# wzhe06/SparrowRecSys

Hardware: AMD Instinct MI355X
Metric: ctr_samples_per_sec (higher is better)
Workload: dtype f32

## Files before the change

### sparrowrecsys_amd/csrc/api_forward.h

```cpp
static int launch_din_cols(sprk_handle h, const int32_t* ids, float* pooled, float* att, int32_t B, const DinColsMany* many, hipStream_t st) {
    DinColsRun c = h->din_cols_run;
    const long long ntasks = (long long)(many ? many->n : 1) * ((B + 15) / 16);
    const long long slots = (long long)h->num_cus * 16;
    c.ts = (c.T >= 16 && ntasks * 4 <= slots) ? 4 : ((c.T >= 8 && ntasks * 2 <= slots) ? 2 : 1);
    if (h->tune.din_cols_ts) c.ts = h->tune.din_cols_ts;
    if (many) c.ts = 1;
    c.ts_log2 = c.ts == 4 ? 2 : (c.ts == 2 ? 1 : 0);
    c.ql = (c.T + 3) / 4;
    const int EL = 4 * h->din_cols_kc;
    const size_t lds = ((size_t)2 * 64 * 36 + (size_t)DC_WAVES * 16 * c.idp + (size_t)DC_WAVES * 2 * 64 * EL) * sizeof(float);
    const long long grid = (ntasks * c.ts + DC_WAVES - 1) / DC_WAVES;
    if (many) {
        if (h->din_cols_kc == 2)
            hipLaunchKernelGGL((k_din_attn_cols<2, true>), dim3((unsigned)grid), dim3(DC_WAVES * 64), lds, st, c, (const int*)nullptr, (float*)nullptr, (float*)nullptr, B, h->dev_err, *many);
        else
            hipLaunchKernelGGL((k_din_attn_cols<1, true>), dim3((unsigned)grid), dim3(DC_WAVES * 64), lds, st, c, (const int*)nullptr, (float*)nullptr, (float*)nullptr, B, h->dev_err, *many);
    } else {
        if (h->din_cols_kc == 2)
            hipLaunchKernelGGL((k_din_attn_cols<2, false>), dim3((unsigned)grid), dim3(DC_WAVES * 64), lds, st, c, ids, pooled, att, B, h->dev_err, DinColsOne{});
        else
            hipLaunchKernelGGL((k_din_attn_cols<1, false>), dim3((unsigned)grid), dim3(DC_WAVES * 64), lds, st, c, ids, pooled, att, B, h->dev_err, DinColsOne{});
    }
    HIP_TRY(hipGetLastError());
    return SPRK_OK;
}

static int launch_din_fused(sprk_handle h, const int32_t* ids, const float* dense, float* out, float* att, int32_t B, const DinFusedMany* many,
                            bool tail, hipStream_t st) {
    DinFusedRun c = h->din_fused_run;
    const long long ntasks = (long long)(many ? many->n : 1) * ((B + 15) / 16);
    const long long slots = (long long)h->num_cus * DF_WAVES;
    c.ts = (c.T >= 16 && ntasks * 4 <= slots) ? 4 : ((c.T >= 8 && ntasks * 2 <= slots) ? 2 : 1);
    if (h->tune.din_cols_ts) c.ts = h->tune.din_cols_ts;
    c.ts_log2 = c.ts == 4 ? 2 : (c.ts == 2 ? 1 : 0);
    c.ql = ((c.T + 3) / 4 + 3) & ~3;
    const int kc = h->din_cols_kc;
    const size_t lds = ((size_t)DF_COEF_FLOATS + (tail ? (size_t)DinFusedImg::dma_floats : 0) + (size_t)DF_WAVES * 16 * c.idp +
                        (size_t)DF_WAVES * (tail ? 1 : 2) * 64 * 4 * kc) * sizeof(float);
    long long grid = (ntasks * c.ts + DF_WAVES - 1) / DF_WAVES;
    if (many && grid > h->num_cus) grid = h->num_cus;
#define DF_LAUNCH(KC, MB, TAIL, marg)                                                                                                   \
    hipLaunchKernelGGL((k_din_fused<KC, MB, TAIL>), dim3((unsigned)grid), dim3(DF_WAVES * 64), lds, st, c, MB ? (const int*)nullptr : ids, \
                       MB ? (const float*)nullptr : dense, MB ? (float*)nullptr : out, MB ? (float*)nullptr : att, B, h->dev_err, marg)
    if (many) {
        if (kc == 2) { if (tail) DF_LAUNCH(2, true, true, *many); else DF_LAUNCH(2, true, false, *many); }
        else { if (tail) DF_LAUNCH(1, true, true, *many); else DF_LAUNCH(1, true, false, *many); }
    } else {
        if (att && !tail) {
            if (kc == 2) hipLaunchKernelGGL((k_din_fused<2, false, false, true>), dim3((unsigned)grid), dim3(DF_WAVES * 64), lds, st, c, ids, dense, out, att, B, h->dev_err, DinFusedOne{});
            else hipLaunchKernelGGL((k_din_fused<1, false, false, true>), dim3((unsigned)grid), dim3(DF_WAVES * 64), lds, st, c, ids, dense, out, att, B, h->dev_err, DinFusedOne{});
        } else if (kc == 2) { if (tail) DF_LAUNCH(2, false, true, DinFusedOne{}); else DF_LAUNCH(2, false, false, DinFusedOne{}); }
        else { if (tail) DF_LAUNCH(1, false, true, DinFusedOne{}); else DF_LAUNCH(1, false, false, DinFusedOne{}); }
    }
#undef DF_LAUNCH
    HIP_TRY(hipGetLastError());
    return SPRK_OK;
}

static int launch_din(sprk_handle h, const int32_t* ids, float* pooled, float* att, int32_t B, hipStream_t st) {
    if (att && (h->stage == Stage::DienSeq || h->stage == Stage::DienSeqMfma)) return fail(SPRK_EINVAL, "DIEN stage has no attention output");
    switch (h->stage) {
    case Stage::DinFusedAttn: return launch_din_fused(h, ids, nullptr, pooled, att, B, nullptr, false, st);
    case Stage::DinCols: return launch_din_cols(h, ids, pooled, att, B, nullptr, st);
    case Stage::DinPool: {
        const int nchunks = (B + h->din_ms - 1) / h->din_ms;
        const int grid = nchunks < h->din_grid_cap ? nchunks : h->din_grid_cap;
        hipLaunchKernelGGL(k_din_pool, dim3(grid), dim3(256), h->din_lds_bytes, st, h->dev_plan, ids, pooled, att, B, h->din_ms, h->dev_err);
        break;
    }
    case Stage::DienSeqMfma: {
        DienRun run = h->dien_run;
        run.image = h->dien_frag;
        const int ntiles = (B + 15) / 16;
        int gridm = (ntiles + DM_WAVES - 1) / DM_WAVES;
        if (gridm > h->num_cus * 8) gridm = h->num_cus * 8;
        const size_t lds10 = DienFrag<10, 32>::total_pad * sizeof(float), lds16 = DienFrag<16, 32>::total_pad * sizeof(float);
        if (h->plan.din.emb_dim == 10)
            hipLaunchKernelGGL((k_dien_seq_mfma<10, 32>), dim3(gridm), dim3(DM_WAVES * 64), lds10, st, run, ids, pooled, B, h->dev_err);
        else
            hipLaunchKernelGGL((k_dien_seq_mfma<16, 32>), dim3(gridm), dim3(DM_WAVES * 64), lds16, st, run, ids, pooled, B, h->dev_err);
        break;
    }
    case Stage::DienSeq: {
        int grid = (B + 63) / 64;
        if (grid > h->num_cus * 8) grid = h->num_cus * 8;
        if (h->plan.din.emb_dim == 10)
            hipLaunchKernelGGL((k_dien_seq<10, 32>), dim3(grid), dim3(64), 0, st, h->dien_run, ids, pooled, B, h->dev_err);
        else
            hipLaunchKernelGGL((k_dien_seq<16, 32>), dim3(grid), dim3(64), 0, st, h->dien_run, ids, pooled, B, h->dev_err);
        break;
    }
    case Stage::None: return fail(SPRK_EKIND, "handle has no DIN stage");
    }
    HIP_TRY(hipGetLastError());
    return SPRK_OK;
}

static int din_tail_waves(sprk_handle h) {
    return h->din_tail_run.e_unscale != 0.f ? dt_waves_unf(kDinTailVariants[h->din_tail_variant].kpc) : DT_WAVES;
}

int sprk_din_pool(sprk_handle h, const int32_t* ids, float* pooled, float* att, int32_t B, void* stream) {
    RoctxRange roctx_range_("sprk_din_pool");
    if (!h || !ids || !pooled) return fail(SPRK_EINVAL, "NULL argument");
    if (!h->finalized) return fail(SPRK_ESTATE, "din_pool before finalize");
    if (!h->plan.din.enabled) return fail(SPRK_EKIND, "handle has no DIN stage");
    if (B <= 0) return B == 0 ? SPRK_OK : fail(SPRK_EINVAL, "negative batch");
    return launch_din(h, ids, pooled, att, B, (hipStream_t)stream);
}

int sprk_forward(sprk_handle h, const int32_t* ids, const float* dense, float* out, int32_t B,
                 void* workspace, size_t workspace_bytes, void* stream) {
    RoctxRange roctx_range_("sprk_forward");
    if (!h) return fail(SPRK_EINVAL, "handle is NULL");
    if (!h->finalized) return fail(SPRK_ESTATE, "forward before finalize");
    if (B < 0) return fail(SPRK_EINVAL, "negative batch");
    if (B == 0) return SPRK_OK;
    if (!out) return fail(SPRK_EINVAL, "out is NULL");
    if (h->plan.n_id_cols > 0 && !ids) return fail(SPRK_EINVAL, "ids is NULL");
    if (h->plan.n_dense > 0 && !dense) return fail(SPRK_EINVAL, "dense is NULL");
    hipStream_t st = (hipStream_t)stream;
    const float* aux = nullptr;
    if (h->plan.din.enabled) {
        const size_t need = sprk_workspace_bytes(h, B);
        if (!workspace || workspace_bytes < need) return fail(SPRK_EINVAL, "workspace too small: %zu < %zu bytes", workspace_bytes, need);
        if (h->route == Route::DinFused) {
            if ((long long)((B + 15) / 16) <= (long long)h->num_cus * DF_WAVES) return launch_din_fused(h, ids, dense, out, nullptr, B, nullptr, true, st);
            DinFusedMany fm;
            memset(&fm, 0, sizeof(fm));
            fm.n = 1; fm.ids[0] = ids; fm.dense[0] = dense; fm.out[0] = out;
            return launch_din_fused(h, nullptr, nullptr, nullptr, nullptr, B, &fm, true, st);
        }
        if (h->route == Route::DienFused) {
            DienRun run = h->dien_run;
            run.image = h->dien_frag;
            const int ntiles = (B + 15) / 16;
            int grid = (ntiles + DNF_WAVES - 1) / DNF_WAVES;
            if (grid > h->num_cus) grid = h->num_cus;
            if (h->plan.din.emb_dim == 10)
                hipLaunchKernelGGL((k_dien_fused<10, 32, 8, 4>), dim3(grid), dim3(DNF_WAVES * 64), h->dien_fused_lds, st, run, h->din_tail_run, ids, dense, out, B,
                                   h->dev_err, (const float*)h->din_tail_image, (float*)workspace);
            else
                hipLaunchKernelGGL((k_dien_fused<16, 32, 8, 4>), dim3(grid), dim3(DNF_WAVES * 64), h->dien_fused_lds, st, run, h->din_tail_run, ids, dense, out, B,
                                   h->dev_err, (const float*)h->din_tail_image, (float*)workspace);
            HIP_TRY(hipGetLastError());
            return SPRK_OK;
        }
        SPRK_TRY(launch_din(h, ids, (float*)workspace, nullptr, B, st));
        aux = (const float*)workspace;
    }
    const int ntasks = (B + 15) / 16;
    const int unaligned = (((uintptr_t)ids | (uintptr_t)dense) & 15) ? 1 : 0;
    switch (h->route) {
    case Route::V2Joint: {
        const V2JVariant& jv = kV2JVariants[h->v2j_variant];
        V2JRun jr = h->v2j_run;
        jr.flags = unaligned;
        const V2J1Variant* one = nullptr;
        if (h->v2j1_image && ntasks <= V2J1_MAX_TASKS)
            for (const V2J1Variant& v : kV2J1Variants)
                if (!one && v.g_big == jv.g_big && v.njf == jv.njf) one = &v;
        if (one) {
            (h->v2j1_hoist ? one->launch_h : one->launch)(jr, ids, dense, out, B, h->dev_err, h->v2j1_image, (ntasks + h->v2j1_waves - 1) / h->v2j1_waves,
                                                          h->v2j1_lds_bytes, st);
            break;
        }
        int grid = (ntasks + V2_WAVES - 1) / V2_WAVES;
        if (grid > h->v2_grid_cap) grid = h->v2_grid_cap;
        jv.launch(jr, ids, dense, out, B, h->dev_err, h->v2_image, grid, h->v2j_lds_bytes, st);
        break;
    }
    case Route::Rows: {
        int grid = (ntasks + RC_WAVES - 1) / RC_WAVES;
        if (grid > h->num_cus) grid = h->num_cus;
        RowsRun rr = h->rows_run;
        rr.flags = unaligned;
        if (h->rows_one && ntasks <= V2J1_MAX_TASKS)
            kRowsVariants[h->rows_variant].launch_one(rr, ids, dense, out, B, h->dev_err, h->rows_image, (ntasks + RC_WAVES - 1) / RC_WAVES,
                                                      h->rows_lds_bytes, st);
        else
            kRowsVariants[h->rows_variant].launch(rr, ids, dense, out, B, h->dev_err, h->rows_image, grid, h->rows_lds_bytes, st);
        break;
    }
    case Route::Pairs: {
        int grid = (ntasks + V1_WAVES - 1) / V1_WAVES;
        if (grid > h->num_cus) grid = h->num_cus;
        if (h->v1_one && ntasks <= V1_ONE_MAX_TASKS)
            kV1Variants[h->v1_variant].launch_one(h->v1_run, ids, dense, out, B, h->dev_err, (ntasks + V1_WAVES - 1) / V1_WAVES, st);
        else
            kV1Variants[h->v1_variant].launch(h->v1_run, ids, dense, out, B, h->dev_err, grid, st);
        break;
    }
    case Route::MlpRows: {
        int grid = (ntasks + MR_WAVES - 1) / MR_WAVES;
        if (grid > h->num_cus) grid = h->num_cus;
        MlpRowsRun rr = h->mlp_rows_run;
        rr.flags = (rr.flags & ~1) | unaligned;
        hipLaunchKernelGGL(h->mlp_rows_kernel, dim3(grid), dim3(MR_WAVES * 64), h->mlp_rows_lds, st, rr, ids, dense, out, B, h->dev_err, (const float*)h->mlp_rows_image);
        break;
    }
    case Route::DinTail: {
        const int tw = din_tail_waves(h);
        int grid = (ntasks + tw - 1) / tw;
        if (grid > h->num_cus) grid = h->num_cus;
        kDinTailVariants[h->din_tail_variant].launch(h->din_tail_run, ids, dense, aux, out, B, h->dev_err, h->din_tail_image, grid, st);
        break;
    }
    default: {
        const int ntiles = (B + SPRK_TILE_M - 1) / SPRK_TILE_M;
        const int grid = ntiles < h->tile_grid_cap ? ntiles : h->tile_grid_cap;
        hipLaunchKernelGGL(k_tile_forward, dim3(grid), dim3(256), h->tile_lds_bytes, st, h->dev_plan, ids, dense, aux, out, B, h->dev_err);
    }
    }
    HIP_TRY(hipGetLastError());
    return SPRK_OK;
}

static int fork_helpers(sprk_handle h, int S, hipStream_t st) {
    HIP_TRY(hipEventRecord(h->many_fork, st));
    for (int s = 0; s < S; ++s) HIP_TRY(hipStreamWaitEvent(h->many_stream[s], h->many_fork, 0));
    return SPRK_OK;
}
static int join_helpers(sprk_handle h, int S, hipStream_t st) {
    for (int s = 0; s < S; ++s) {
        HIP_TRY(hipEventRecord(h->many_join[s], h->many_stream[s]));
        HIP_TRY(hipStreamWaitEvent(st, h->many_join[s], 0));
    }
    return SPRK_OK;
}

extern "C++" {
template <class Many, class Launch>
static int launch_groups(int32_t n_batches, int per, const int32_t* const* ids, const float* const* dense, float* const* out, Launch launch) {
    int g = 0;
    for (int32_t i0 = 0; i0 < n_batches; i0 += per, ++g) {
        Many m;
        memset(&m, 0, sizeof(m));
        m.n = n_batches - i0 < per ? n_batches - i0 : per;
        for (int j = 0; j < m.n; ++j) { m.ids[j] = ids[i0 + j]; m.dense[j] = dense ? dense[i0 + j] : nullptr; m.out[j] = out[i0 + j]; }
        SPRK_TRY(launch(m, g));
        HIP_TRY(hipGetLastError());
    }
    return SPRK_OK;
}
template <class Ok> static bool every_batch(int32_t n_batches, Ok ok) {
    for (int32_t i = 0; i < n_batches; ++i)
        if (!ok(i)) return false;
    return true;
}
}

static int forward_many_impl(sprk_handle h, int32_t n_batches, const int32_t* const* ids, const float* const* dense,
                             float* const* out, int32_t B, void* workspace, size_t workspace_bytes, void* stream,
                             int many_batches, int many_streams) {
    RoctxRange roctx_range_("sprk_forward_many");
    if (!h) return fail(SPRK_EINVAL, "handle is NULL");
    if (n_batches < 0) return fail(SPRK_EINVAL, "negative batch count");
    if (n_batches > 0 && !out) return fail(SPRK_EINVAL, "out is NULL");
    int S = (h->finalized && n_batches > 1) ? many_streams : 0;
    const size_t ws_need = (sprk_workspace_bytes(h, B) + 255) & ~(size_t)255;
    const bool ws_untouched = h->finalized && (h->route == Route::DinFused || h->route == Route::DienFused);
    if (S >= 2 && ws_need > 0 && !ws_untouched) {
        while (S >= 2 && (!workspace || workspace_bytes < (size_t)S * ws_need)) --S;
        if (S < 2) S = 0;
    }
    hipStream_t st = (hipStream_t)stream;
    const bool grouped = h->finalized && many_batches > 1 && n_batches > 1 && B > 0 && ids;
    const int ntpb = (B + 15) / 16;
    auto aligned = [&](int32_t i, const float* d) { return !(((uintptr_t)ids[i] | (uintptr_t)d) & 15); };
    auto present = [&](int32_t i) { return ids[i] && dense[i] && out[i]; };
    if (grouped && dense && h->route == Route::V2Joint && every_batch(n_batches, [&](int32_t i) { return present(i) && aligned(i, dense[i]); })) {
        const V2JVariant& jv = kV2JVariants[h->v2j_variant];
        V2JRun jr = h->v2j_run;
        jr.flags = 0;
        return launch_groups<V2JMany>(n_batches, many_batches, ids, dense, out, [&](V2JMany& m, int) {
            m.ntpb = ntpb;
            long long grid = ((long long)m.n * ntpb + V2_WAVES - 1) / V2_WAVES;
            if (grid > h->v2_grid_cap) grid = h->v2_grid_cap;
            jv.launch_many(jr, m, B, h->dev_err, h->v2_image, (int)grid, h->v2j_lds_bytes, st);
            return SPRK_OK;
        });
    }
    const float* const* rows_dense = h->plan.n_dense ? dense : nullptr;
    if (grouped && (dense || h->plan.n_dense == 0) && h->route == Route::Rows &&
        every_batch(n_batches, [&](int32_t i) { return ids[i] && out[i] && (!rows_dense || rows_dense[i]) && aligned(i, rows_dense ? rows_dense[i] : nullptr); })) {
        const RowsVariant& rv = kRowsVariants[h->rows_variant];
        RowsRun rr = h->rows_run;
        rr.flags = 0;
        return launch_groups<RowsMany>(n_batches, many_batches < RC_MB ? many_batches : RC_MB, ids, rows_dense, out, [&](RowsMany& m, int) {
            m.ntpb = ntpb;
            long long grid = ((long long)m.n * ntpb + RC_WAVES - 1) / RC_WAVES;
            if (grid > h->num_cus) grid = h->num_cus;
            rv.launch_many(rr, m, B, h->dev_err, h->rows_image, (int)grid, h->rows_lds_bytes, st);
            return SPRK_OK;
        });
    }
    if (grouped && dense && h->route == Route::MlpRows && h->mlp_rows_many_kernel &&
        every_batch(n_batches, [&](int32_t i) { return present(i) && aligned(i, dense[i]); })) {
        MlpRowsRun rr = h->mlp_rows_run;
        rr.flags &= ~1;
        return launch_groups<MlpRowsMany>(n_batches, many_batches < MR_MB ? many_batches : MR_MB, ids, dense, out, [&](MlpRowsMany& m, int) {
            long long grid = ((long long)m.n * ntpb + MR_WAVES - 1) / MR_WAVES;
            if (grid > h->num_cus) grid = h->num_cus;
            hipLaunchKernelGGL(h->mlp_rows_many_kernel, dim3((int)grid), dim3(MR_WAVES * 64), h->mlp_rows_lds, st, rr, m, B, h->dev_err,
                               (const float*)h->mlp_rows_image);
            return SPRK_OK;
        });
    }
    if (grouped && dense && h->route == Route::Pairs && every_batch(n_batches, present)) {
        const V1Variant& vv = kV1Variants[h->v1_variant];
        return launch_groups<V1Many>(n_batches, many_batches < V1_MB ? many_batches : V1_MB, ids, dense, out, [&](V1Many& m, int) {
            m.ntpb = ntpb;
            long long grid = ((long long)m.n * ntpb + V1_WAVES - 1) / V1_WAVES;
            if (grid > h->num_cus) grid = h->num_cus;
            vv.launch_many(h->v1_run, m, B, h->dev_err, (int)grid, st);
            return SPRK_OK;
        });
    }
    if (grouped && dense && h->route == Route::DinFused && h->tune.din_fused_mb && every_batch(n_batches, present)) {
        const int SG = S >= 2 ? S : 1;
        if (SG >= 2) SPRK_TRY(fork_helpers(h, SG, st));
        SPRK_TRY(launch_groups<DinFusedMany>(n_batches, many_batches < DF_MB ? many_batches : DF_MB, ids, dense, out, [&](DinFusedMany& m, int g) {
            return launch_din_fused(h, nullptr, nullptr, nullptr, nullptr, B, &m, true, SG >= 2 ? h->many_stream[g % SG] : st);
        }));
        if (SG >= 2) SPRK_TRY(join_helpers(h, SG, st));
        return SPRK_OK;
    }
    const bool cols = h->stage == Stage::DinCols || h->stage == Stage::DinFusedAttn;
    if (grouped && dense && workspace && ws_need > 0 && cols && (h->route == Route::DinTail || h->route == Route::DinFused)) {
        int per = many_batches < DIN_MB ? many_batches : DIN_MB;
        if ((size_t)per * ws_need > workspace_bytes) per = (int)(workspace_bytes / ws_need);
        if (per >= 2 && every_batch(n_batches, present)) {
            int SG = S >= 2 ? S : 1;
            while (SG > 1 && (size_t)SG * per * ws_need > workspace_bytes) --SG;
            if (SG >= 2) SPRK_TRY(fork_helpers(h, SG, st));
            const DinTailVariant& tv = kDinTailVariants[h->din_tail_variant];
            const int tw = din_tail_waves(h);
            int g = 0;
            for (int32_t i0 = 0; i0 < n_batches; i0 += per, ++g) {
                const int n = n_batches - i0 < per ? n_batches - i0 : per;
                hipStream_t sg = SG >= 2 ? h->many_stream[g % SG] : st;
                char* wbase = (char*)workspace + (size_t)(g % SG) * per * ws_need;
                DinTailMany tm;
                memset(&tm, 0, sizeof(tm));
                tm.n = n; tm.ntpb = ntpb;
                for (int j = 0; j < n; ++j) {
                    float* pooled = (float*)(wbase + (size_t)j * ws_need);
                    tm.ids[j] = ids[i0 + j]; tm.dense[j] = dense[i0 + j]; tm.aux[j] = pooled; tm.out[j] = out[i0 + j];
                }
                if (n <= DC_MB) {
                    DinColsMany cm;
                    memset(&cm, 0, sizeof(cm));
                    cm.n = n;
                    for (int j = 0; j < n; ++j) { cm.ids[j] = tm.ids[j]; cm.pooled[j] = const_cast<float*>(tm.aux[j]); }
                    SPRK_TRY(launch_din_cols(h, nullptr, nullptr, nullptr, B, &cm, sg));
                } else {
                    for (int j = 0; j < n; ++j) SPRK_TRY(launch_din_cols(h, tm.ids[j], const_cast<float*>(tm.aux[j]), nullptr, B, nullptr, sg));
                }
                long long tg = ((long long)n * ntpb + tw - 1) / tw;
                if (tg > h->num_cus) tg = h->num_cus;
                tv.launch_many(h->din_tail_run, tm, B, h->dev_err, h->din_tail_image, (int)tg, sg);
                HIP_TRY(hipGetLastError());
            }
            if (SG >= 2) SPRK_TRY(join_helpers(h, SG, st));
            return SPRK_OK;
        }
    }
    if (S >= 2) SPRK_TRY(fork_helpers(h, S, st));
    for (int32_t i = 0; i < n_batches; ++i) {
        const bool sliced = S >= 2 && ws_need > 0 && !ws_untouched;
        void* wsi = sliced ? (void*)((char*)workspace + (size_t)(i % S) * ws_need) : workspace;
        SPRK_TRY(sprk_forward(h, ids ? ids[i] : nullptr, dense ? dense[i] : nullptr, out[i], B, wsi,
                              sliced ? ws_need : workspace_bytes, S >= 2 ? (void*)h->many_stream[i % S] : stream));
    }
    if (S >= 2) SPRK_TRY(join_helpers(h, S, st));
    return SPRK_OK;
}

int sprk_forward_many(sprk_handle h, int32_t n_batches, const int32_t* const* ids, const float* const* dense,
                      float* const* out, int32_t B, void* workspace, size_t workspace_bytes, void* stream) {
    if (!h) return fail(SPRK_EINVAL, "handle is NULL");
    return forward_many_impl(h, n_batches, ids, dense, out, B, workspace, workspace_bytes, stream, h->many_batches, h->many_streams);
}

int sprk_forward_many_opts(sprk_handle h, int32_t n_batches, const int32_t* const* ids, const float* const* dense,
                           float* const* out, int32_t B, void* workspace, size_t workspace_bytes, void* stream,
                           int32_t batches_per_launch, int32_t helper_streams) {
    if (!h) return fail(SPRK_EINVAL, "handle is NULL");
    if (batches_per_launch < 1 || batches_per_launch > V2J_MB) return fail(SPRK_EINVAL, "batches per launch %d outside [1,%d]", batches_per_launch, V2J_MB);
    if (helper_streams < 0 || helper_streams > 4) return fail(SPRK_EINVAL, "stream count %d outside [0,4]", helper_streams);
    return forward_many_impl(h, n_batches, ids, dense, out, B, workspace, workspace_bytes, stream, batches_per_launch,
                             helper_streams < 2 ? 0 : helper_streams);
}

#define SPRK_FORWARD_KIND(name, kind)                                                                      \
    int name(sprk_handle h, const int32_t* ids, const float* dense, float* out, int32_t B, void* ws,      \
             size_t ws_bytes, void* stream) {                                                              \
        if (!h) return fail(SPRK_EINVAL, "handle is NULL");                                                \
        if (h->plan.model_kind != kind) return fail(SPRK_EKIND, #name ": handle holds model kind %d", h->plan.model_kind); \
        return sprk_forward(h, ids, dense, out, B, ws, ws_bytes, stream);                                  \
    }
SPRK_FORWARD_KIND(sprk_forward_embedding_mlp, SPRK_MODEL_EMBEDDING_MLP)
SPRK_FORWARD_KIND(sprk_forward_widedeep, SPRK_MODEL_WIDE_DEEP)
SPRK_FORWARD_KIND(sprk_forward_neuralcf, SPRK_MODEL_NEURALCF)
SPRK_FORWARD_KIND(sprk_forward_deepfm, SPRK_MODEL_DEEPFM)
SPRK_FORWARD_KIND(sprk_forward_deepfm_v2, SPRK_MODEL_DEEPFM_V2)
SPRK_FORWARD_KIND(sprk_forward_din, SPRK_MODEL_DIN)
SPRK_FORWARD_KIND(sprk_forward_dien, SPRK_MODEL_DIEN)

int sprk_set_many_streams(sprk_handle h, int32_t n) {
    if (!h) return fail(SPRK_EINVAL, "handle is NULL");
    if (!h->finalized) return fail(SPRK_ESTATE, "set_many_streams before finalize");
    if (n < 0 || n > 4) return fail(SPRK_EINVAL, "stream count %d outside [0,4]", n);
    h->many_streams = n < 2 ? 0 : n;
    return SPRK_OK;
}

int sprk_set_many_batches(sprk_handle h, int32_t n) {
    if (!h) return fail(SPRK_EINVAL, "handle is NULL");
    if (!h->finalized) return fail(SPRK_ESTATE, "set_many_batches before finalize");
    if (n < 1 || n > V2J_MB) return fail(SPRK_EINVAL, "batches per launch %d outside [1,%d]", n, V2J_MB);
    h->many_batches = n;
    return SPRK_OK;
}

int sprk_describe(sprk_handle h, char* buf, size_t buf_bytes) {
    if (!h || !buf || buf_bytes == 0) return fail(SPRK_EINVAL, "describe: NULL argument");
    if (!h->finalized) return fail(SPRK_ESTATE, "describe before finalize");
    char kern[160];
    switch (h->route) {
    case Route::V2Joint: {
        const V2JVariant& jv = kV2JVariants[h->v2j_variant];
        snprintf(kern, sizeof(kern), "k_deepfm_v2_joint<G_BIG=%d,NJF=%d,KPC=%d,%s>", jv.g_big, jv.njf, jv.kpc, jv.half ? "split-f16" : "f32");
        break;
    }
    case Route::Pairs:
        snprintf(kern, sizeof(kern), "k_deepfm_pairs<NF=%d,NV=%d>", kV1Variants[h->v1_variant].nf, kV1Variants[h->v1_variant].nv);
        break;
    case Route::Rows: {
        const RowsVariant& rv = kRowsVariants[h->rows_variant];
        snprintf(kern, sizeof(kern), "k_rows_chain<KPC=%d,H0C=%d,H1C=%d,G_BIG=%d,NJF=%d%s>", rv.kpc, rv.h0c, rv.h1c, rv.g_big, rv.njf,
                 rv.unf ? ",UNF" : "");
        break;
    }
    case Route::MlpRows:
        snprintf(kern, sizeof(kern), "k_mlp_rows<8,8,NBIG=%d,NSMALL=%d>", h->mlp_rows_nbig, h->mlp_rows_run.n_small);
        break;
    case Route::DinTail: {
        const DinTailVariant& tv = kDinTailVariants[h->din_tail_variant];
        snprintf(kern, sizeof(kern), "k_din_tail<%d,%d,%d%s>", tv.n0c, tv.n1c, tv.kpc, h->din_tail_run.e_unscale != 0.f ? ",UNF" : "");
        break;
    }
    case Route::DinFused: snprintf(kern, sizeof(kern), "k_din_fused<KC=%d,tail 128/64>", h->din_cols_kc); break;
    case Route::DienFused: snprintf(kern, sizeof(kern), "k_dien_fused<D=%d,tail 128/64>", h->plan.din.emb_dim); break;
    case Route::Tile: snprintf(kern, sizeof(kern), "k_tile_forward"); break;
    }
    static const char* const kStageName[] = {"", "k_din_pool", "k_din_attn_cols", "k_din_fused", "k_dien_seq", "k_dien_seq_mfma"};
    const bool cols = h->stage == Stage::DinCols || h->stage == Stage::DinFusedAttn;
    size_t uploaded = 0;
    for (size_t b : h->slot_bytes) uploaded += b;
#ifndef SPRK_BUILD_DEFINES_STR
#define SPRK_BUILD_DEFINES_STR ""
#endif
    char split[96] = "";
    auto site = [&](bool on, const char* name) {
        if (!on) return;
        if (split[0]) strncat(split, ",", sizeof(split) - strlen(split) - 1);
        strncat(split, name, sizeof(split) - strlen(split) - 1);
    };
    switch (h->route) {
    case Route::V2Joint: site(kV2JVariants[h->v2j_variant].half, "v2"); break;
    case Route::Pairs:
        site(h->v1_run.w1frag != nullptr, "dyn_w1"); site(h->v1_run.w0frag != nullptr, "dyn_w0"); site(h->v1_run.e_scale != 0.f, "pairs_e");
        break;
    case Route::Rows: site(kRowsVariants[h->rows_variant].unf, "rows_unf"); break;
    case Route::MlpRows: site(h->mlp_rows_run.inv_w1_scale != 0.f, "dyn_w1"); break;
    case Route::DinTail: case Route::DinFused: case Route::DienFused:
        site(h->din_tail_run.inv_w1_scale != 0.f, "dyn_w1"); site(h->din_tail_run.inv_w0p_scale != 0.f, "dyn_w0p");
        site(h->din_tail_run.e_unscale != 0.f, "tail_unf");
        break;
    case Route::Tile: break;
    }
    site(cols, "din_attn");
    site(h->stage == Stage::DienSeqMfma, "dien_seq");
    const int n = snprintf(buf, buf_bytes, "kernel=%s;stage=%s;stage_waves_per_workgroup=%d;fused=%d;uploaded_bytes=%zu;derived_bytes=%zu;first_dense_fold=%d;split_f16=%s;build_defines=%s", kern,
                           kStageName[(int)h->stage], cols ? DC_WAVES : 0, h->route != Route::Tile ? 1 : 0, uploaded, h->derived_bytes, h->n_acc_folded, split, SPRK_BUILD_DEFINES_STR);
    if (n < 0 || (size_t)n >= buf_bytes) return fail(SPRK_EINVAL, "describe: buffer of %zu bytes is too small", buf_bytes);
    return SPRK_OK;
}

int sprk_check_ids(sprk_handle h, void* stream) {
    if (!h) return fail(SPRK_EINVAL, "handle is NULL");
    if (!h->finalized) return fail(SPRK_ESTATE, "check_ids before finalize");
    int flag = 0;
    HIP_TRY(hipMemcpyAsync(&flag, h->dev_err, sizeof(int), hipMemcpyDeviceToHost, (hipStream_t)stream));
    HIP_TRY(hipStreamSynchronize((hipStream_t)stream));
    if (flag) {
        HIP_TRY(hipMemsetAsync(h->dev_err, 0, sizeof(int), (hipStream_t)stream));
        HIP_TRY(hipStreamSynchronize((hipStream_t)stream));
        return fail(SPRK_ERANGE, "an id was outside its table (TF would raise InvalidArgumentError: assert_less_than_num_buckets) [flag 0x%x]", flag);
    }
    return SPRK_OK;
}

void sprk_destroy(sprk_handle h) {
    if (!h) return;
    for (size_t i = 0; i < h->slot_ptr.size(); ++i) free_slot(h, i);
    for (const sprk_engine::DevAlloc& a : h->allocs) release(a);
    if (h->v2j_tab) (void)hipFree(h->v2j_tab);
    for (int i = 0; i < 4; ++i) { if (h->many_stream[i]) (void)hipStreamDestroy(h->many_stream[i]); if (h->many_join[i]) (void)hipEventDestroy(h->many_join[i]); }
    if (h->many_fork) (void)hipEventDestroy(h->many_fork);
    delete h;
}

int sprk_embedding_gather(const float* table, int32_t V, int32_t D, int32_t row_stride, const int32_t* ids,
                          int32_t B, float* out, void* stream) {
    if (!table || !ids || !out) return fail(SPRK_EINVAL, "NULL argument");
    if (V <= 0 || D <= 0 || (D & 3) || row_stride < D || (row_stride & 3)) return fail(SPRK_EINVAL, "bad gather geometry V=%d D=%d row_stride=%d", V, D, row_stride);
    if (B < 0) return fail(SPRK_EINVAL, "negative batch");
    if (B == 0) return SPRK_OK;
    const long long total = (long long)B * (D / 4);
    long long blocks = (total + 255) / 256;
    if (blocks > 8192) blocks = 8192;
    hipLaunchKernelGGL(k_embedding_gather, dim3((unsigned)blocks), dim3(256), 0, (hipStream_t)stream, table, V, D / 4, row_stride, ids, B, out);
    HIP_TRY(hipGetLastError());
    return SPRK_OK;
}
```

### sparrowrecsys_amd/csrc/host_common.h

```cpp
#pragma GCC visibility push(hidden)
namespace sprk_dev {

typedef float f32x4 __attribute__((ext_vector_type(4)));

inline thread_local std::string g_err;

inline int fail(int code, const char* fmt, ...) {
    char buf[512];
    va_list ap;
    va_start(ap, fmt);
    vsnprintf(buf, sizeof(buf), fmt, ap);
    va_end(ap);
    g_err = buf;
    return code;
}

#define HIP_TRY(expr)                                                                      \
    do {                                                                                   \
        hipError_t e_ = (expr);                                                            \
        if (e_ != hipSuccess) return fail(SPRK_EHIP, "%s failed: %s", #expr, hipGetErrorString(e_)); \
    } while (0)
#define SPRK_TRY(expr)                                                                     \
    do {                                                                                   \
        if (const int rc_ = (expr)) return rc_;                                            \
    } while (0)

template <class T> struct DevScratch {
    T* p = nullptr;
    DevScratch() = default;
    ~DevScratch() { if (p) (void)hipFree(p); }
    hipError_t alloc(size_t n) { return hipMalloc((void**)&p, n * sizeof(T)); }
    DevScratch(const DevScratch&) = delete;
    DevScratch& operator=(const DevScratch&) = delete;
};

struct Roctx {
    int (*push)(const char*) = nullptr;
    int (*pop)() = nullptr;
    bool on = false;
    Roctx() {
        const char* e = getenv("SPRK_ROCTX");
        if (!e || e[0] != '1') return;
        void* lib = nullptr;
        for (const char* n : {"librocprofiler-sdk-roctx.so.1", "librocprofiler-sdk-roctx.so", "libroctx64.so.4", "libroctx64.so"}) {
            lib = dlopen(n, RTLD_NOW | RTLD_GLOBAL);
            if (lib) break;
        }
        if (!lib) return;
        push = reinterpret_cast<int (*)(const char*)>(dlsym(lib, "roctxRangePushA"));
        pop = reinterpret_cast<int (*)()>(dlsym(lib, "roctxRangePop"));
        on = push && pop;
    }
};
inline const Roctx& roctx() { static const Roctx r; return r; }
struct RoctxRange {
    bool live;
    explicit RoctxRange(const char* name) : live(roctx().on) { if (live) roctx().push(name); }
    ~RoctxRange() { if (live) roctx().pop(); }
    RoctxRange(const RoctxRange&) = delete;
    RoctxRange& operator=(const RoctxRange&) = delete;
};

struct SprkTuning {
    bool force_interpreter = false;
    bool v2_fold = true;
    bool v2_rows = false;
    bool v2_joint = true;
    bool v2_half = true;
    bool v2j_one = true;
    int v2j1_hoist = -1;
    bool tail_unf = true;
    bool tail_pooled_f16 = true;
    bool dien_mfma = true;
    bool rows_unf = true;
    bool ncf_chain = true;
    bool tile_fold = true;
    bool half_range_guard = true;
    bool dyn_f16 = true;
    bool v1_chain = true;
    bool v1_one = true;
    bool mlp_chain = true;
    bool vmm_tables = true;
    bool din_tail = true;
    bool din_legacy = false;
    bool din_half = true;
    bool din_cols = true;
    bool din_fused = true;
    bool din_fused_mb = true;
    bool din_fused_unf = true;
    bool dien_fused = true;
    int din_fused_min_t = 12;
    bool mlp_rows_many = true;
    int din_cols_ts = 0;
    int many_streams = 0;
    static SprkTuning from_env() {
        auto off = [](const char* n) { const char* e = getenv(n); return e && e[0] == '0'; };
        auto on = [](const char* n) { const char* e = getenv(n); return e && e[0] == '1'; };
        auto num = [](const char* n, int dflt) { const char* e = getenv(n); return e ? atoi(e) : dflt; };
        SprkTuning t;
        t.force_interpreter = on("SPRK_FORCE_INTERPRETER");
        t.v2_fold = !off("SPRK_V2_FOLD"); t.v2_rows = on("SPRK_V2_ROWS"); t.v2_joint = !off("SPRK_V2_JOINT"); t.v2_half = !off("SPRK_V2_HALF");
        t.v2j_one = !off("SPRK_V2J_ONE"); t.v2j1_hoist = num("SPRK_V2J1_HOIST", -1);
        t.rows_unf = !off("SPRK_ROWS_UNF"); t.dien_mfma = !off("SPRK_DIEN_MFMA"); t.tail_pooled_f16 = !off("SPRK_TAIL_POOLED_F16"); t.tail_unf = !off("SPRK_TAIL_UNF"); t.ncf_chain = !off("SPRK_NCF_CHAIN"); t.tile_fold = !off("SPRK_TILE_FOLD");
        t.half_range_guard = !off("SPRK_HALF_RANGE_GUARD"); t.dyn_f16 = !off("SPRK_DYN_F16");
        t.v1_chain = !off("SPRK_V1_CHAIN");
        t.v1_one = !off("SPRK_V1_ONE");
        t.mlp_chain = !off("SPRK_MLP_CHAIN");
        t.vmm_tables = !off("SPRK_VMM_TABLES");
        t.din_tail = !off("SPRK_DIN_TAIL"); t.din_legacy = on("SPRK_DIN_LEGACY"); t.din_half = !off("SPRK_DIN_HALF");
        t.din_cols = !off("SPRK_DIN_COLS"); t.din_fused = !off("SPRK_DIN_FUSED"); t.mlp_rows_many = !off("SPRK_MLP_ROWS_MANY"); t.din_fused_mb = !off("SPRK_DIN_FUSED_MB"); t.din_fused_unf = !off("SPRK_DIN_FUSED_UNF"); t.din_fused_min_t = num("SPRK_DIN_FUSED_MIN_T", 12); t.dien_fused = !off("SPRK_DIEN_FUSED");
        { const int n = num("SPRK_DIN_COLS_TS", 0); t.din_cols_ts = (n == 1 || n == 2 || n == 4) ? n : 0; }
        { const int n = num("SPRK_MANY_STREAMS", 0); t.many_streams = n < 2 ? 0 : (n > 4 ? 4 : n); }
        return t;
    }
};
inline thread_local const SprkTuning* g_finalize_tune = nullptr;
```

### sparrowrecsys_amd/csrc/host_setup_pairs.h

```cpp
constexpr int V1_WAVES = 8;
constexpr int V1_ONE_MAX_TASKS = 16384;
typedef void (*V1LaunchFn)(const V1Run&, const int*, const float*, float*, int, int*, int, hipStream_t);
typedef void (*V1LaunchManyFn)(const V1Run&, const V1Many&, int, int*, int, hipStream_t);
template <int NF, int NV, bool SEP>
void v1_launch(const V1Run& a, const int* ids, const float* dense, float* out, int B, int* err, int grid, hipStream_t st) {
    const size_t lds = V1Lds<4, 4, (NV + 3) / 4>::bytes;
    if (a.inv_w1_scale != 0.f)
        hipLaunchKernelGGL((k_deepfm_pairs<NF, NV, 4, 4, V1_WAVES, true, SEP>), dim3(grid), dim3(V1_WAVES * 64), lds, st, a, ids, dense, out, B, err);
    else
        hipLaunchKernelGGL((k_deepfm_pairs<NF, NV, 4, 4, V1_WAVES, false, SEP>), dim3(grid), dim3(V1_WAVES * 64), lds, st, a, ids, dense, out, B, err);
}
template <int NF, int NV, bool SEP>
void v1_launch_one(const V1Run& a, const int* ids, const float* dense, float* out, int B, int* err, int grid, hipStream_t st) {
    if constexpr (NV <= 4) {
        const size_t lds = V1Lds<4, 4, 1>::bytes;
        hipLaunchKernelGGL((k_deepfm_pairs1<NF, NV, 4, 4, V1_WAVES, SEP>), dim3(grid), dim3(V1_WAVES * 64), lds, st, a, ids, dense, out, B, err);
    }
}
template <int NF, int NV, bool SEP>
void v1_launch_many(const V1Run& a, const V1Many& m, int B, int* err, int grid, hipStream_t st) {
    const size_t lds = V1Lds<4, 4, (NV + 3) / 4>::bytes;
    if (a.inv_w1_scale != 0.f)
        hipLaunchKernelGGL((k_deepfm_pairs_many<NF, NV, 4, 4, V1_WAVES, true, SEP>), dim3(grid), dim3(V1_WAVES * 64), lds, st, a, m, B, err);
    else
        hipLaunchKernelGGL((k_deepfm_pairs_many<NF, NV, 4, 4, V1_WAVES, false, SEP>), dim3(grid), dim3(V1_WAVES * 64), lds, st, a, m, B, err);
}
template <int NF, int NV, bool SEP>
int v1_prepare(const V1Run& r, float* img) {
    constexpr int PC = (NV + 3) / 4;
    hipLaunchKernelGGL((k_v1_pack_image<4, 4, PC>), dim3(1), dim3(256), 0, 0, r, img);
    HIP_TRY(hipGetLastError());
    const size_t lds = V1Lds<4, 4, PC>::bytes;
    HIP_TRY(hipFuncSetAttribute(reinterpret_cast<const void*>(&k_deepfm_pairs<NF, NV, 4, 4, V1_WAVES, true, SEP>), hipFuncAttributeMaxDynamicSharedMemorySize, (int)lds));
    HIP_TRY(hipFuncSetAttribute(reinterpret_cast<const void*>(&k_deepfm_pairs<NF, NV, 4, 4, V1_WAVES, false, SEP>), hipFuncAttributeMaxDynamicSharedMemorySize, (int)lds));
    HIP_TRY(hipFuncSetAttribute(reinterpret_cast<const void*>(&k_deepfm_pairs_many<NF, NV, 4, 4, V1_WAVES, true, SEP>), hipFuncAttributeMaxDynamicSharedMemorySize, (int)lds));
    HIP_TRY(hipFuncSetAttribute(reinterpret_cast<const void*>(&k_deepfm_pairs_many<NF, NV, 4, 4, V1_WAVES, false, SEP>), hipFuncAttributeMaxDynamicSharedMemorySize, (int)lds));
    if constexpr (NV <= 4)
        HIP_TRY(hipFuncSetAttribute(reinterpret_cast<const void*>(&k_deepfm_pairs1<NF, NV, 4, 4, V1_WAVES, SEP>), hipFuncAttributeMaxDynamicSharedMemorySize, (int)lds));
    return SPRK_OK;
}
struct V1Variant { int nf, nv; bool sep; V1LaunchFn launch; V1LaunchFn launch_one; V1LaunchManyFn launch_many; int (*prepare)(const V1Run&, float*); size_t lds_bytes; };
#define V1_VARIANT(NF, NV, SEP) {NF, NV, SEP, &v1_launch<NF, NV, SEP>, &v1_launch_one<NF, NV, SEP>, &v1_launch_many<NF, NV, SEP>, &v1_prepare<NF, NV, SEP>, V1Lds<4, 4, (NV + 3) / 4>::bytes}
#define V1_BOTH(NF, NV) V1_VARIANT(NF, NV, true), V1_VARIANT(NF, NV, false)
const V1Variant kV1Variants[] = {
    V1_BOTH(6, 4),
    V1_BOTH(4, 3),
    V1_BOTH(4, 4),
    V1_BOTH(4, 16),
};

int setup_deepfm_pairs(sprk_engine* h) {
    if (!h->tune.v1_chain) return SPRK_OK;
    const sprk_plan& p = h->plan;
    if (p.model_kind != SPRK_MODEL_DEEPFM || p.din.enabled || p.n_ops != 3 || p.n_taps != 3 || p.n_pairs < 1) return SPRK_OK;
    const sprk_op &od = p.ops[0], &o0 = p.ops[1], &o1 = p.ops[2];
    if (od.kind != SPRK_OP_PAIR_DOT || od.src_buf != 0 || od.dst_buf != 0) return SPRK_OK;
    if (o0.kind != SPRK_OP_DENSE || o0.act != SPRK_ACT_RELU || o0.src_buf != 0 || o0.dst_buf != 1 || o0.dst_off != 0 || o0.N != 64) return SPRK_OK;
    if (o1.kind != SPRK_OP_DENSE || o1.act != SPRK_ACT_RELU || o1.src_buf != 1 || o1.src_off != 0 || o1.K != o0.N || o1.dst_off != 0 || o1.N != 64) return SPRK_OK;
    V1Run r;
    memset(&r, 0, sizeof(r));
    int row_dst[V1_MAX_FIELDS], nf = 0, Dp = 0, num_dst = -1, scal_dst[V1_MAX_FIELDS], ns = 0, scal_col[V1_MAX_FIELDS], scal_vocab[V1_MAX_FIELDS];
    const float* scal_tab[V1_MAX_FIELDS];
    const int ds0 = o0.src_off, ds1 = o0.src_off + o0.K;
    int dsep_col[V1_MAX_DEEP], dsep_vocab[V1_MAX_DEEP], dsep_dst[V1_MAX_DEEP], n_dsep = 0;
    const float* dsep_tab[V1_MAX_DEEP];
    for (int i = 0; i < p.n_segs; ++i) {
        const sprk_seg& sg = p.segs[i];
        if (sg.kind == SPRK_SEG_ROWS) {
            if (nf == 0 && n_dsep == 0) Dp = sg.row_stride;
            if (sg.row_stride != Dp || sg.count * 4 != Dp || Dp > 64) return SPRK_OK;
            if (h->slot_bytes[sg.slot] < ((size_t)sg.vocab + 1) * Dp * sizeof(float)) return SPRK_OK;
            bool twin_outside = false;
            for (int j = 0; j < p.n_segs; ++j)
                if (j != i && p.segs[j].kind == SPRK_SEG_ROWS && p.segs[j].field == sg.field &&
                    !(p.segs[j].dst >= ds0 && p.segs[j].dst + p.segs[j].row_stride <= ds1)) twin_outside = true;
            if (twin_outside && sg.dst >= ds0 && sg.dst + Dp <= ds1) {
                if (n_dsep == V1_MAX_DEEP) return SPRK_OK;
                dsep_col[n_dsep] = sg.field; dsep_vocab[n_dsep] = sg.vocab; dsep_tab[n_dsep] = (const float*)h->slot_ptr[sg.slot];
                dsep_dst[n_dsep++] = sg.dst;
                continue;
            }
            if (nf == V1_MAX_FIELDS) return SPRK_OK;
            r.col[nf] = sg.field; r.vocab[nf] = sg.vocab; r.table[nf] = (const float*)h->slot_ptr[sg.slot];
            row_dst[nf++] = sg.dst;
        } else if (sg.kind == SPRK_SEG_SCALAR) {
            if (ns == V1_MAX_FIELDS) return SPRK_OK;
            if (h->slot_bytes[sg.slot] < ((size_t)sg.vocab + 1) * sizeof(float)) return SPRK_OK;
            scal_col[ns] = sg.field; scal_vocab[ns] = sg.vocab; scal_tab[ns] = (const float*)h->slot_ptr[sg.slot]; scal_dst[ns++] = sg.dst;
        } else if (sg.kind == SPRK_SEG_DENSE) {
            if (num_dst >= 0 || sg.field != 0 || sg.count > 8) return SPRK_OK;
            num_dst = sg.dst; r.n_num = sg.count;
        } else if (sg.kind != SPRK_SEG_ZERO) {
            return SPRK_OK;
        }
    }
    if (nf < 2 || ns != nf || num_dst < 0 || r.n_num < 1) return SPRK_OK;
    for (int f = 0; f < nf; ++f) {
        int hit = -1;
        for (int i = 0; i < ns; ++i) if (scal_col[i] == r.col[f] && scal_vocab[i] == r.vocab[f]) hit = i;
        if (hit < 0) return SPRK_OK;
        r.w1[f] = scal_tab[hit];
    }
    int smin = scal_dst[0];
    for (int i = 1; i < ns; ++i) if (scal_dst[i] < smin) smin = scal_dst[i];
    const sprk_tap *tf = nullptr, *tpair = nullptr, *tdeep = nullptr;
    for (int t = 0; t < 3; ++t) {
        const sprk_tap& tp = p.taps[t];
        if (tp.scale != 1.0f || tp.bias != 0.0f) return SPRK_OK;
        if (tp.buf == 0 && tp.off == smin && tp.len == ns && tp.w_slot < 0) tf = &tp;
        else if (tp.buf == 0 && tp.off == od.dst_off && tp.len == p.n_pairs && tp.w_slot >= 0) tpair = &tp;
        else if (tp.buf == o1.dst_buf && tp.off == 0 && tp.len <= o1.N && tp.w_slot >= 0) tdeep = &tp;
    }
    if (!tf || !tpair || !tdeep) return SPRK_OK;
    for (int i = 0; i < ns; ++i) if (scal_dst[i] < smin || scal_dst[i] >= smin + ns) return SPRK_OK;
    std::vector<float> pwh(p.n_pairs);
    HIP_TRY(hipMemcpy(pwh.data(), h->slot_ptr[tpair->w_slot], p.n_pairs * sizeof(float), hipMemcpyDeviceToHost));
    for (int i = 0; i < p.n_pairs; ++i) {
        int a = -1, b = -1;
        for (int f = 0; f < nf; ++f) { if (row_dst[f] == p.pair_a[i]) a = f; if (row_dst[f] == p.pair_b[i]) b = f; }
        if (a < 0 || b < 0 || a == b || od.K != Dp) return SPRK_OK;
        if (a > b) { const int t = a; a = b; b = t; }
        r.pw[a * V1_MAX_FIELDS + b] += pwh[i];
    }
    const int s0 = ds0, s1 = ds1;
    if (num_dst < s0 || num_dst + r.n_num > s1) return SPRK_OK;
    int order[V1_MAX_FIELDS], no = 0, deep_off[V1_MAX_DEEP] = {0, 0};
    const bool sep = n_dsep > 0;
    for (int f = 0; f < nf; ++f) {
        if (row_dst[f] >= s0 && row_dst[f] + Dp <= s1) {
            if (sep || r.n_deep == V1_MAX_DEEP) return SPRK_OK;
            deep_off[r.n_deep++] = row_dst[f] - s0;
            order[no++] = f;
        } else if (row_dst[f] < s1 && row_dst[f] + Dp > s0) {
            return SPRK_OK;
        }
    }
    if (sep) {
        for (int d = 0; d < n_dsep; ++d) {
            int twin = -1;
            for (int f = 0; f < nf; ++f) if (r.col[f] == dsep_col[d] && r.vocab[f] == dsep_vocab[d]) twin = f;
            if (twin < 0) return SPRK_OK;
            for (int i = 0; i < no; ++i) if (order[i] == twin) return SPRK_OK;
            deep_off[r.n_deep++] = dsep_dst[d] - s0;
            order[no++] = twin;
        }
    }
    for (int f = 0; f < nf; ++f) {
        bool deep = false;
        for (int i = 0; i < r.n_deep; ++i) deep |= order[i] == f;
        if (!deep) order[no++] = f;
    }
    {
        V1Run t = r;
        int inv[V1_MAX_FIELDS];
        for (int i = 0; i < nf; ++i) {
            const int f = order[i];
            inv[f] = i;
            t.col[i] = r.col[f]; t.vocab[i] = r.vocab[f]; t.table[i] = r.table[f]; t.w1[i] = r.w1[f];
        }
        memset(t.pw, 0, sizeof(t.pw));
        for (int a = 0; a < nf; ++a)
            for (int b = a + 1; b < nf; ++b) {
                const float w = r.pw[a * V1_MAX_FIELDS + b];
                if (w == 0.f) continue;
                int x = inv[a], y = inv[b];
                if (x > y) { const int tt = x; x = y; y = tt; }
                t.pw[x * V1_MAX_FIELDS + y] += w;
            }
        r = t;
    }
    r.sep = sep ? 1 : 0;
    for (int d = 0; d < n_dsep; ++d) r.table[nf + d] = dsep_tab[d];
    const float* const* deep_tables = sep ? &r.table[nf] : &r.table[0];
    int variant = -1;
    for (size_t v = 0; v < sizeof(kV1Variants) / sizeof(kV1Variants[0]); ++v)
        if (kV1Variants[v].nf == nf && kV1Variants[v].nv == Dp / 4 && kV1Variants[v].sep == sep) variant = (int)v;
    if (variant < 0) return SPRK_OK;
    const int H0 = o0.N, H1 = o1.N;
    const float* W0 = (const float*)h->slot_ptr[o0.w_slot];
    const int PC = (Dp / 4 + 3) / 4;
    const int KW = 16 * (V1_MAX_DEEP * PC + 1);
    float* w0p = nullptr;
    SPRK_TRY(dev_alloc(h, &w0p, (size_t)H0 * KW * sizeof(float) + 16));
    hipLaunchKernelGGL(k_v1_pack_w0, dim3(1), dim3(256), 0, 0, W0, o0.ldw, r.n_deep, deep_off[0], deep_off[1], Dp, num_dst - s0, r.n_num,
                       H0, PC, w0p);
    HIP_TRY(hipGetLastError());
    float* hd = nullptr;
    SPRK_TRY(dev_alloc(h, &hd, (size_t)H1 * sizeof(float) + 16));
    HIP_TRY(hipMemset(hd, 0, (size_t)H1 * sizeof(float)));
    HIP_TRY(hipMemcpy(hd, h->slot_ptr[tdeep->w_slot], (size_t)tdeep->len * sizeof(float), hipMemcpyDeviceToDevice));
    HIP_TRY(hipDeviceSynchronize());
    r.F = p.n_id_cols; r.ND = p.n_dense; r.nf = nf; r.row_floats = Dp;
    r.w0 = w0p; r.b0 = (const float*)h->slot_ptr[o0.b_slot];
    r.W1 = (const float*)h->slot_ptr[o1.w_slot]; r.ld1 = o1.ldw; r.b1 = (const float*)h->slot_ptr[o1.b_slot];
    r.hdeep = hd; r.head_bias = p.head_bias;
    r.w1frag = nullptr; r.inv_w1_scale = 0.f; r.w0frag = nullptr; r.inv_w0_scale = 0.f;
    {
        float w_scale = 0.f, w0_scale = 0.f;
        float *frag = nullptr, *frag0 = nullptr;
        int rc2 = make_dyn_fragments(h, r.W1, r.ld1, H1, H0, &frag, &w_scale);
        if (rc2) return rc2;
        if (frag && (rc2 = make_dyn_fragments(h, w0p, KW, H0, 32 * PC, &frag0, &w0_scale))) return rc2;
        if (frag && frag0) { r.w1frag = frag; r.inv_w1_scale = 1.0f / w_scale; r.w0frag = frag0; r.inv_w0_scale = 1.0f / w0_scale; }
    }
    {
        float* img = nullptr;
        SPRK_TRY(dev_alloc(h, &img, kV1Variants[variant].lds_bytes));
        SPRK_TRY(kV1Variants[variant].prepare(r, img));
        HIP_TRY(hipDeviceSynchronize());
        r.image = img;
    }
    r.e_scale = 0.f; r.e_inv = 0.f;
    {
        if (r.w0frag) {
            std::vector<AbsmaxJob> jobs;
            for (int f = 0; f < r.n_deep; ++f) {
                const long long rows = (long long)r.vocab[f] + 1;
                jobs.push_back({deep_tables[f], rows, Dp, Dp, absmax_grid(rows * Dp, 8192), 0});
            }
            float mx = 0.f;
            SPRK_TRY(device_absmax(jobs, &mx, 1));
            bool wide = false;
            for (int f = 0; f < r.n_deep && !wide && mx > 0.f && mx < 3.0e38f; ++f)
                SPRK_TRY(wide_dynamic_range(deep_tables[f], (long long)r.vocab[f] + 1, Dp, Dp, mx, &wide));
            if (mx > 0.f && mx < 3.0e38f && !wide) {
                r.e_scale = pow2_scale(mx);
                r.e_inv = r.inv_w0_scale / r.e_scale;
            }
        }
    }
    r.tab = nullptr;
    if (PC == 1) {
        const int pack = !sep ? 0 : (Dp <= 12 ? 80 : (Dp == 16 ? 64 : 0));
        size_t rows = 0;
        for (int f = 0; f < nf; ++f) rows += (size_t)r.vocab[f] + 1;
        if (sep && !pack) for (int d = 0; d < r.n_deep; ++d) rows += (size_t)r.vocab[d] + 1;
        if (rows * 128 < ((size_t)1 << 32)) {
            float* tab = nullptr;
            SPRK_TRY(table_alloc(h, &tab, rows * 128));
            h->derived_bytes += rows * 128;
            float* w1c = nullptr;
            if (pack == 64) {
                size_t nw = 0;
                for (int d = 0; d < r.n_deep; ++d) { r.w1cbase[d] = (unsigned)nw; nw += (size_t)r.vocab[d] + 1; }
                SPRK_TRY(dev_alloc(h, &w1c, nw * sizeof(float) + 16));
                for (int d = 0; d < r.n_deep; ++d)
                    HIP_TRY(hipMemcpy(w1c + r.w1cbase[d], r.w1[d], ((size_t)r.vocab[d] + 1) * sizeof(float), hipMemcpyDeviceToDevice));
            }
            size_t base = 0;
            for (int f = 0; f < nf + ((sep && !pack) ? r.n_deep : 0); ++f) {
                const bool deep_row = f >= nf;
                const bool packed_here = pack && f < r.n_deep;
                const long long n = (long long)r.vocab[deep_row ? f - nf : f] + 1;
                long long nb = (n * 32 + 255) / 256;
                if (nb > 65536) nb = 65536;
                hipLaunchKernelGGL(k_v1_build_rows, dim3((unsigned)nb), dim3(256), 0, 0, r.table[f], Dp,
                                   (deep_row || (packed_here && pack == 64)) ? (const float*)nullptr : r.w1[f], n, tab + base * 32,
                                   packed_here ? r.table[nf + f] : (const float*)nullptr, pack / 4);
                r.rowbase[f] = (unsigned)base;
                base += (size_t)n;
            }
            HIP_TRY(hipGetLastError());
            HIP_TRY(hipDeviceSynchronize());
            r.tab = tab;
            r.pack = pack;
            r.w1c = w1c;
        }
    }
    {
        h->v1_one = r.tab && r.w1frag && PC == 1 && h->tune.v1_one;
    }
    h->v1_run = r;
    h->v1_variant = variant;
    return SPRK_OK;
}
```

### sparrowrecsys_amd/csrc/k_chain_v1.h

```cpp

#define V1_MAX_FIELDS 8
#define V1_MAX_DEEP 2
#define V1_MAX_ROWS (V1_MAX_FIELDS + V1_MAX_DEEP)

struct V1Run {
    int F, ND, n_num;
    int nf;
    int col[V1_MAX_FIELDS];
    int vocab[V1_MAX_FIELDS];
    int row_floats;
    const float* table[V1_MAX_ROWS];
    const float* w1[V1_MAX_FIELDS];
    int n_deep;
    int sep;
    int pack;
    const float* w1c;
    unsigned w1cbase[V1_MAX_DEEP];
    float pw[V1_MAX_FIELDS * V1_MAX_FIELDS];
    const float* w0;
    const float* b0;
    const float* W1;
    int ld1;
    const float* b1;
    const float* hdeep;
    float head_bias;
    const float* w1frag;
    float inv_w1_scale;
    const float* w0frag;
    float inv_w0_scale;
    const float* image;
    float e_scale, e_inv;
    const float* tab;
    unsigned rowbase[V1_MAX_ROWS];
};

static __global__ __launch_bounds__(256) void k_v1_build_rows(const float* __restrict__ table, int Dp, const float* __restrict__ w1,
                                                       long long rows, float* __restrict__ out, const float* __restrict__ deep, int deep_off) {
    const long long total = rows * 32;
    for (long long i = (long long)blockIdx.x * 256 + threadIdx.x; i < total; i += (long long)gridDim.x * 256) {
        const long long v = i >> 5;
        const int c = (int)(i & 31);
        float x = c < Dp ? table[v * Dp + c] : ((c == 16 && w1) ? w1[v] : 0.f);
        if (deep && c >= deep_off && c - deep_off < Dp) x = deep[v * Dp + (c - deep_off)];
        out[i] = x;
    }
}

static __global__ __launch_bounds__(256) void k_v1_pack_w0(const float* __restrict__ W0, int ldw0, int n_deep, int off0, int off1,
                                                    int Dp, int n_off, int n_num, int H0, int PC, float* __restrict__ w0) {
    const int KW = 16 * (V1_MAX_DEEP * PC + 1);
    for (int i = threadIdx.x; i < H0 * KW; i += 256) {
        const int n = i / KW, k = i - n * KW, c = k >> 4, j = k & 15;
        float v = 0.f;
        if (c < V1_MAX_DEEP * PC) {
            const int f = c / PC, col = 16 * (c - f * PC) + j;
            if (f < n_deep && col < Dp) v = W0[(size_t)n * ldw0 + (f == 0 ? off0 : off1) + col];
        } else if (j < n_num) {
            v = W0[(size_t)n * ldw0 + n_off + j];
        }
        w0[i] = v;
    }
}

#define V1_MB 16
struct V1Many {
    const int* ids[V1_MB];
    const float* dense[V1_MB];
    float* out[V1_MB];
    int n, ntpb;
};

template <int H0C, int H1C, int PC = 1>
struct V1Lds {
    static constexpr int H0 = H0C * 16, H1 = H1C * 16;
    static constexpr int S1 = H0 + 4;
    static constexpr int KE = 32 * PC;
    static constexpr int SE = KE + 4;
    static constexpr int off_w1 = 0;
    static constexpr int off_w0e = off_w1 + H1 * S1;
    static constexpr int off_w0n = off_w0e + H0 * SE;
    static constexpr int off_b0 = off_w0n + H0 * 8;
    static constexpr int off_b1 = off_b0 + H0;
    static constexpr int off_hd = off_b1 + H1;
    static constexpr int total = off_hd + H1;
    static constexpr int total_pad = (total + 255) & ~255;
    static constexpr size_t bytes = sizeof(float) * total_pad;
    static_assert(H1C * (H0C / 2) * 512 <= H1 * S1 && H0C * PC * 512 <= H0 * SE && H0C % 2 == 0, "fragments fit their regions");
};

template <int H0C, int H1C, int PC>
__global__ __launch_bounds__(256) void k_v1_pack_image(const V1Run A, float* __restrict__ img) {
    using LD = V1Lds<H0C, H1C, PC>;
    const int tid = threadIdx.x, KW = 16 * (V1_MAX_DEEP * PC + 1);
    for (int i = tid; i < LD::total_pad; i += 256) img[i] = 0.f;
    __syncthreads();
    if (A.w1frag) {
        for (int i = tid; i < H1C * (H0C / 2) * 512; i += 256) img[LD::off_w1 + i] = A.w1frag[i];
    } else {
        for (int i = tid; i < LD::H1 * LD::S1; i += 256) {
            const int n = i / LD::S1, k = i - n * LD::S1;
            img[LD::off_w1 + i] = k < LD::H0 ? A.W1[(size_t)n * A.ld1 + k] : 0.f;
        }
    }
    if (A.w0frag) {
        for (int i = tid; i < H0C * PC * 512; i += 256) img[LD::off_w0e + i] = A.w0frag[i];
    } else {
        for (int i = tid; i < LD::H0 * LD::SE; i += 256) {
            const int n = i / LD::SE, k = i - n * LD::SE;
            img[LD::off_w0e + i] = k < LD::KE ? A.w0[(size_t)n * KW + k] : 0.f;
        }
    }
    for (int i = tid; i < LD::H0 * 8; i += 256) img[LD::off_w0n + i] = A.w0[(size_t)(i >> 3) * KW + 16 * V1_MAX_DEEP * PC + (i & 7)];
    for (int i = tid; i < LD::H0; i += 256) img[LD::off_b0 + i] = A.b0[i];
    for (int i = tid; i < LD::H1; i += 256) { img[LD::off_b1 + i] = A.b1[i]; img[LD::off_hd + i] = A.hdeep[i]; }
}

template <int NR, int PC>
struct V1Set {
    f32x4 x[NR][PC];
    float xa, xb;
    float w1a, w1b;
};

template <int NF, int NV, int H0C, int H1C, int WAVES, bool DYN, bool MB, bool SEP, bool ONE = false>
__device__ __forceinline__ void v1_body(const V1Run& A, const int* __restrict__ ids0, const float* __restrict__ dense0,
                                        float* __restrict__ out0, int B, int* __restrict__ err, const V1Many* __restrict__ Mp) {
    constexpr int PC = (NV + 3) / 4;
    constexpr int NR = NF + (SEP ? V1_MAX_DEEP : 0);
    constexpr int DB = SEP ? NF : 0;
    using LD = V1Lds<H0C, H1C, PC>;
    using Set = V1Set<NR, PC>;
    static_assert(!(ONE && MB) && !(ONE && PC > 1), "one-task shape: one batch, narrow rows");
    static_assert(NF >= 2 && NF <= V1_MAX_FIELDS && NV >= 1 && (NV <= 4 || NV % 4 == 0) && NV <= 16, "shape");
    const int tid = threadIdx.x;
    const int lane = tid & 63;
    const int wave = __builtin_amdgcn_readfirstlane(tid >> 6);
    const int r = lane & 15, q = lane >> 4;
    const f32x4 zero = f32x4{0.f, 0.f, 0.f, 0.f};
    const int m_ntpb = MB ? Mp->ntpb : 0;
    const int ntasks = MB ? Mp->n * m_ntpb : (B + 15) >> 4;
    const int task_stride = gridDim.x * WAVES;
    bool bad = false;
    auto batch_of = [&](int t, int& tl) {
        if constexpr (MB) {
            const int b = __builtin_amdgcn_readfirstlane(t / m_ntpb);
            tl = t - b * m_ntpb;
            return b;
        } else {
            tl = t;
            return 0;
        }
    };
    auto ld_ids = [&](int tg, int (&idv)[NF]) {
        int t;
        const int bi = batch_of(tg, t);
        const int* ids = MB ? Mp->ids[bi] : ids0;
        const int m = min(t * 16 + r, B - 1);
        const int* row = ids + (size_t)m * A.F;
#pragma unroll
        for (int f = 0; f < NF; ++f) idv[f] = row[A.col[f]];
    };
    auto issue_gather = [&](int tg, const int (&idv)[NF], Set& S) {
        int t;
        const int bi = batch_of(tg, t);
        const float* dense = MB ? Mp->dense[bi] : dense0;
        const int m = min(t * 16 + r, B - 1);
        {
            const float* nrow = dense + (size_t)m * A.ND;
            const int last = A.n_num - 1;
            S.xa = nrow[min(q, last)];
            S.xb = nrow[min(q + 4, last)];
        }
        unsigned sid[NF];
#pragma unroll
        for (int f = 0; f < NF; ++f) {
            bad |= (unsigned)(idv[f] + 1) > (unsigned)A.vocab[f];
            sid[f] = min((unsigned)idv[f], (unsigned)A.vocab[f]);
        }
        if ((ONE && NV == 4) || (PC == 1 && A.tab)) {
            const char* tb = reinterpret_cast<const char*>(A.tab);
            unsigned ro[NF];
#pragma unroll
            for (int f = 0; f < NF; ++f) ro[f] = (sid[f] + A.rowbase[f]) * 128u;
#pragma unroll
            for (int f = 0; f < NF; ++f) S.x[f][0] = q < NV ? *reinterpret_cast<const f32x4*>(tb + (ro[f] + 16u * q)) : zero;
            if constexpr (SEP) {
#pragma unroll
                for (int d = 0; d < V1_MAX_DEEP; ++d) {
                    S.x[NF + d][0] = zero;
                    if (d < A.n_deep) {
                        const unsigned rd = A.pack ? ro[d] + (unsigned)A.pack : (sid[d] + A.rowbase[NF + d]) * 128u;
                        if (q < NV) S.x[NF + d][0] = *reinterpret_cast<const f32x4*>(tb + (rd + 16u * q));
                    }
                }
            }
            unsigned oa = ro[0], ob = ro[NF > 4 ? 4 : 0];
            if (NF > 1) oa = q == 1 ? ro[NF > 1 ? 1 : 0] : oa;
            if (NF > 2) oa = q == 2 ? ro[NF > 2 ? 2 : 0] : oa;
            if (NF > 3) oa = q == 3 ? ro[NF > 3 ? 3 : 0] : oa;
            if (NF > 5) ob = q == 1 ? ro[NF > 5 ? 5 : 0] : ob;
            if (NF > 6) ob = q == 2 ? ro[NF > 6 ? 6 : 0] : ob;
            if (NF > 7) ob = q == 3 ? ro[NF > 7 ? 7 : 0] : ob;
            const float* pa = reinterpret_cast<const float*>(tb + (oa + 64u));
            if (A.w1c) {
                const unsigned ci = (q == 1 ? sid[1] + A.w1cbase[1] : sid[0] + A.w1cbase[0]);
                pa = q < A.n_deep ? A.w1c + ci : pa;
            }
            S.w1a = (q < NF) ? *pa : 0.f;
            S.w1b = (NF > 4 && q + 4 < NF) ? *reinterpret_cast<const float*>(tb + (ob + 64u)) : 0.f;
            return;
        }
#pragma unroll
        for (int f = 0; f < NF; ++f)
#pragma unroll
            for (int pc = 0; pc < PC; ++pc)
                S.x[f][pc] = 4 * pc + q < NV ? ld4(A.table[f] + (size_t)sid[f] * A.row_floats + 16 * pc + 4 * q) : zero;
        if constexpr (SEP) {
#pragma unroll
            for (int d = 0; d < V1_MAX_DEEP; ++d)
#pragma unroll
                for (int pc = 0; pc < PC; ++pc)
                    S.x[NF + d][pc] = (d < A.n_deep && 4 * pc + q < NV) ? ld4(A.table[NF + d] + (size_t)sid[d] * A.row_floats + 16 * pc + 4 * q) : zero;
        }
        {
            const float* pa = A.w1[0] + sid[0];
            if (NF > 1) pa = q == 1 ? A.w1[NF > 1 ? 1 : 0] + sid[NF > 1 ? 1 : 0] : pa;
            if (NF > 2) pa = q == 2 ? A.w1[NF > 2 ? 2 : 0] + sid[NF > 2 ? 2 : 0] : pa;
            if (NF > 3) pa = q == 3 ? A.w1[NF > 3 ? 3 : 0] + sid[NF > 3 ? 3 : 0] : pa;
            S.w1a = (q < NF) ? *pa : 0.f;
            S.w1b = 0.f;
            if (NF > 4) {
                const float* pb = A.w1[NF > 4 ? 4 : 0] + sid[NF > 4 ? 4 : 0];
                if (NF > 5) pb = q == 1 ? A.w1[NF > 5 ? 5 : 0] + sid[NF > 5 ? 5 : 0] : pb;
                if (NF > 6) pb = q == 2 ? A.w1[NF > 6 ? 6 : 0] + sid[NF > 6 ? 6 : 0] : pb;
                if (NF > 7) pb = q == 3 ? A.w1[NF > 7 ? 7 : 0] + sid[NF > 7 ? 7 : 0] : pb;
                S.w1b = (q + 4 < NF) ? *pb : 0.f;
            }
        }
    };
    float rna[H0C], rnb[H0C];
    auto compute = [&](const Set& S) -> float {
#pragma clang fp contract(off)
        constexpr bool NUM_FIRST = ONE && NV == 4;
        f32x4 h0[H0C];
        auto deep0_numerics = [&]() {
#pragma unroll
            for (int nb = 0; nb < H0C; ++nb) h0[nb] = ld4(smem + LD::off_b0 + nb * 16 + 4 * q);
#pragma unroll
            for (int nb = 0; nb < H0C; ++nb) h0[nb] = __builtin_amdgcn_mfma_f32_16x16x4f32(rna[nb], S.xa, h0[nb], 0, 0, 0);
#pragma unroll
            for (int nb = 0; nb < H0C; ++nb) h0[nb] = __builtin_amdgcn_mfma_f32_16x16x4f32(rnb[nb], S.xb, h0[nb], 0, 0, 0);
        };
        if constexpr (NUM_FIRST) deep0_numerics();
        typedef float f32x2 __attribute__((ext_vector_type(2)));
        f32x2 pa = {0.f, 0.f}, pb = {0.f, 0.f};
#pragma unroll
        for (int a = 0; a < NF; ++a)
#pragma unroll
            for (int b = a + 1; b < NF; ++b) {
                const float hw = A.pw[a * V1_MAX_FIELDS + b];
                if (hw == 0.f) continue;
                const f32x2 hw2 = {hw, hw};
#pragma unroll
                for (int pc = 0; pc < PC; ++pc) {
                    const f32x4 xa = S.x[a][pc], xb = S.x[b][pc];
                    pa = __builtin_elementwise_fma(f32x2{xa.x, xa.y} * f32x2{xb.x, xb.y}, hw2, pa);
                    pb = __builtin_elementwise_fma(f32x2{xa.z, xa.w} * f32x2{xb.z, xb.w}, hw2, pb);
                }
            }
        float z = (S.w1a + S.w1b) + ((pa[0] + pa[1]) + (pb[0] + pb[1]));
        if constexpr (!NUM_FIRST) deep0_numerics();
        f32x4 ec[2 * PC];
#pragma unroll
        for (int c = 0; c < 2 * PC; ++c) ec[c] = (c / PC == 0 || A.n_deep > 1) ? S.x[DB + c / PC][c % PC] : zero;
        if constexpr (DYN) {
            float scale = A.e_scale, inv = A.e_inv;
            if (A.e_scale == 0.f) {
                float mx = 0.f;
#pragma unroll
                for (int c = 0; c < 2 * PC; ++c)
#pragma unroll
                    for (int j = 0; j < 4; ++j) mx = fmaxf(mx, __builtin_fabsf(ec[c][j]));
                mx = rows4_max(mx);
                dyn_scale(mx, A.inv_w0_scale, scale, inv);
            }
            int wfo = LD::off_w0e + lane * 4;
            asm volatile("" : "+v"(wfo));
            f32x4 acc[H0C];
#pragma unroll
            for (int nb = 0; nb < H0C; ++nb) acc[nb] = zero;
#pragma unroll
            for (int b = 0; b < PC; ++b) {
                din_f16x8 bh, bl;
                dyn_split8(ec[2 * b], ec[2 * b + 1], scale, bh, bl);
#pragma unroll
                for (int nb = 0; nb < H0C; ++nb) {
                    const din_f16x8 ah = __builtin_bit_cast(din_f16x8, ld4(smem + wfo + ((nb * PC + b) * 2 + 0) * 256));
                    const din_f16x8 al = __builtin_bit_cast(din_f16x8, ld4(smem + wfo + ((nb * PC + b) * 2 + 1) * 256));
                    acc[nb] = mfma_f16(ah, bh, acc[nb]);
                    acc[nb] = mfma_f16(ah, bl, acc[nb]);
                    acc[nb] = mfma_f16(al, bh, acc[nb]);
                }
            }
#pragma unroll
            for (int nb = 0; nb < H0C; ++nb) h0[nb] = acc[nb] * inv + h0[nb];
        } else {
            int w0o = LD::off_w0e + r * LD::SE + 4 * q;
            asm volatile("" : "+v"(w0o));
#pragma unroll
            for (int c = 0; c < 2 * PC; ++c) {
                f32x4 a[H0C];
#pragma unroll
                for (int nb = 0; nb < H0C; ++nb) a[nb] = ld4(smem + w0o + nb * 16 * LD::SE + 16 * c);
#pragma unroll
                for (int st = 0; st < 4; ++st)
#pragma unroll
                    for (int nb = 0; nb < H0C; ++nb)
                        h0[nb] = __builtin_amdgcn_mfma_f32_16x16x4f32(a[nb][st], ec[c][st], h0[nb], 0, 0, 0);
            }
        }
#pragma unroll
        for (int nb = 0; nb < H0C; ++nb) h0[nb] = relu4_fast(h0[nb]);
        f32x4 h1[H1C];
        if constexpr (DYN) {
            float mx = 0.f;
#pragma unroll
            for (int nb = 0; nb < H0C; ++nb)
#pragma unroll
                for (int j = 0; j < 4; ++j) mx = fmaxf(mx, h0[nb][j]);
            mx = rows4_max(mx);
            float scale, inv;
            dyn_scale(mx, A.inv_w1_scale, scale, inv);
            f32x4 acc[H1C];
#pragma unroll
            for (int n1 = 0; n1 < H1C; ++n1) acc[n1] = zero;
            int wfo = LD::off_w1 + lane * 4;
            asm volatile("" : "+v"(wfo));
#pragma unroll
            for (int b = 0; b < H0C / 2; ++b) {
                din_f16x8 bh, bl;
                dyn_split8(h0[2 * b], h0[2 * b + 1], scale, bh, bl);
#pragma unroll
                for (int n1 = 0; n1 < H1C; ++n1) {
                    const din_f16x8 ah = __builtin_bit_cast(din_f16x8, ld4(smem + wfo + ((n1 * (H0C / 2) + b) * 2 + 0) * 256));
                    const din_f16x8 al = __builtin_bit_cast(din_f16x8, ld4(smem + wfo + ((n1 * (H0C / 2) + b) * 2 + 1) * 256));
                    acc[n1] = mfma_f16(ah, bh, acc[n1]);
                    acc[n1] = mfma_f16(ah, bl, acc[n1]);
                    acc[n1] = mfma_f16(al, bh, acc[n1]);
                }
            }
#pragma unroll
            for (int n1 = 0; n1 < H1C; ++n1) h1[n1] = acc[n1] * inv + ld4(smem + LD::off_b1 + n1 * 16 + 4 * q);
        } else {
#pragma unroll
            for (int n1 = 0; n1 < H1C; ++n1) h1[n1] = ld4(smem + LD::off_b1 + n1 * 16 + 4 * q);
            int w1o = LD::off_w1 + r * LD::S1 + 4 * q;
            asm volatile("" : "+v"(w1o));
#pragma unroll
            for (int c = 0; c < H0C; ++c) {
                f32x4 a[H1C];
#pragma unroll
                for (int n1 = 0; n1 < H1C; ++n1) a[n1] = ld4(smem + w1o + n1 * 16 * LD::S1 + 16 * c);
#pragma unroll
                for (int st = 0; st < 4; ++st)
#pragma unroll
                    for (int n1 = 0; n1 < H1C; ++n1)
                        h1[n1] = __builtin_amdgcn_mfma_f32_16x16x4f32(a[n1][st], h0[c][st], h1[n1], 0, 0, 0);
            }
        }
#pragma unroll
        for (int n1 = 0; n1 < H1C; ++n1) {
            const f32x4 hd = ld4(smem + LD::off_hd + n1 * 16 + 4 * q), hr = relu4_fast(h1[n1]);
#pragma unroll
            for (int j = 0; j < 4; ++j) z = fmaf(hd[j], hr[j], z);
        }
        z = rows4_sum(z);
        return sigmoidf_acc(z + A.head_bias);
    };
    auto store = [&](int tg, float score) {
        int tl;
        const int bo = batch_of(tg, tl);
        float* out = MB ? Mp->out[bo] : out0;
        const int mm = tl * 16 + r;
        if (q == 0 && mm < B) out[mm] = score;
    };

    int tA = blockIdx.x * WAVES + wave, tB = tA + task_stride;
    int idA[NF], idB[NF];
#pragma unroll
    for (int f = 0; f < NF; ++f) { idA[f] = -1; idB[f] = -1; }
    if (tA < ntasks) ld_ids(tA, idA);
    if (!ONE && tB < ntasks) ld_ids(tB, idB);
#pragma unroll 1
    for (int c = wave; c < LD::total_pad / 256; c += WAVES) lds_dma16(A.image + c * 256 + lane * 4, smem + c * 256);
    Set SA, SB;
    if constexpr (ONE) {
        __builtin_amdgcn_s_waitcnt(0x0F70);
        __builtin_amdgcn_s_barrier();
        if (tA < ntasks) issue_gather(tA, idA, SA);
#pragma unroll
        for (int nb = 0; nb < H0C; ++nb) {
            rna[nb] = smem[LD::off_w0n + (nb * 16 + r) * 8 + q];
            rnb[nb] = smem[LD::off_w0n + (nb * 16 + r) * 8 + q + 4];
        }
        if (tA < ntasks) store(tA, compute(SA));
    } else {
    __builtin_amdgcn_s_waitcnt(0x0F70);
    __builtin_amdgcn_s_barrier();
#pragma unroll
    for (int nb = 0; nb < H0C; ++nb) {
        rna[nb] = smem[LD::off_w0n + (nb * 16 + r) * 8 + q];
        rnb[nb] = smem[LD::off_w0n + (nb * 16 + r) * 8 + q + 4];
    }
    if (tA >= ntasks) {
    } else if (PC == 1 && ntasks <= 2 * task_stride) {
        issue_gather(tA, idA, SA);
        if (tB < ntasks) issue_gather(tB, idB, SB);
        store(tA, compute(SA));
        if (tB < ntasks) store(tB, compute(SB));
    } else {
        issue_gather(tA, idA, SA);
        for (int tk = tA; tk < ntasks; tk += task_stride) {
            const Set cur = SA;
            if (tk + task_stride < ntasks) {
                issue_gather(tk + task_stride, idB, SA);
                if (tk + 2 * task_stride < ntasks) ld_ids(tk + 2 * task_stride, idB);
            }
            store(tk, compute(cur));
        }
    }
    }
    if (__ballot(bad) != 0 && lane == 0) atomicOr(err, 1);
}

template <int NF, int NV, int H0C, int H1C, int WAVES, bool DYN, bool SEP>
__global__ __launch_bounds__(WAVES * 64, 2) void k_deepfm_pairs(const V1Run A, const int* __restrict__ ids, const float* __restrict__ dense,
                                                                float* __restrict__ out, int B, int* __restrict__ err) {
    v1_body<NF, NV, H0C, H1C, WAVES, DYN, false, SEP>(A, ids, dense, out, B, err, nullptr);
}
template <int NF, int NV, int H0C, int H1C, int WAVES, bool DYN, bool SEP>
__global__ __launch_bounds__(WAVES * 64, 2) void k_deepfm_pairs_many(const V1Run A, const V1Many M, int B, int* __restrict__ err) {
    v1_body<NF, NV, H0C, H1C, WAVES, DYN, true, SEP>(A, nullptr, nullptr, nullptr, B, err, &M);
}
template <int NF, int NV, int H0C, int H1C, int WAVES, bool SEP>
__global__ __launch_bounds__(WAVES * 64, 4) void k_deepfm_pairs1(const V1Run A, const int* __restrict__ ids, const float* __restrict__ dense,
                                                                 float* __restrict__ out, int B, int* __restrict__ err) {
    v1_body<NF, NV, H0C, H1C, WAVES, true, false, SEP, true>(A, ids, dense, out, B, err, nullptr);
}
```

### sparrowrecsys_amd/csrc/tu_instances.h

```cpp
#ifndef SPRK_SINGLE_TU
#ifndef SPRK_TU_FAMILY
#define SPRK_TU_FAMILY 0
#endif
#if SPRK_TU_FAMILY == 1
#define SPRK_INST_1 template
#else
#define SPRK_INST_1 extern template
#endif
#if SPRK_TU_FAMILY == 2
#define SPRK_INST_2 template
#else
#define SPRK_INST_2 extern template
#endif
#if SPRK_TU_FAMILY == 3
#define SPRK_INST_3 template
#else
#define SPRK_INST_3 extern template
#endif
#if SPRK_TU_FAMILY == 4
#define SPRK_INST_4 template
#else
#define SPRK_INST_4 extern template
#endif
#if SPRK_TU_FAMILY == 5
#define SPRK_INST_5 template
#else
#define SPRK_INST_5 extern template
#endif
#if SPRK_TU_FAMILY == 6
#define SPRK_INST_6 template
#else
#define SPRK_INST_6 extern template
#endif
SPRK_INST_1 __global__ void sprk_dev::k_deepfm_v2_joint<1, 1, 1, 2, 1, 8, false>(sprk_dev::V2JRun, int const*, float const*, float*, int, int*, float const*);
SPRK_INST_1 __global__ void sprk_dev::k_deepfm_v2_joint<1, 1, 1, 2, 1, 8, true>(sprk_dev::V2JRun, int const*, float const*, float*, int, int*, float const*);
SPRK_INST_1 __global__ void sprk_dev::k_deepfm_v2_joint<1, 2, 1, 2, 1, 8, false>(sprk_dev::V2JRun, int const*, float const*, float*, int, int*, float const*);
SPRK_INST_1 __global__ void sprk_dev::k_deepfm_v2_joint<1, 2, 1, 2, 1, 8, true>(sprk_dev::V2JRun, int const*, float const*, float*, int, int*, float const*);
SPRK_INST_1 __global__ void sprk_dev::k_deepfm_v2_joint<1, 3, 1, 2, 1, 8, false>(sprk_dev::V2JRun, int const*, float const*, float*, int, int*, float const*);
SPRK_INST_1 __global__ void sprk_dev::k_deepfm_v2_joint<1, 3, 1, 2, 1, 8, true>(sprk_dev::V2JRun, int const*, float const*, float*, int, int*, float const*);
SPRK_INST_1 __global__ void sprk_dev::k_deepfm_v2_joint<2, 1, 1, 2, 1, 8, false>(sprk_dev::V2JRun, int const*, float const*, float*, int, int*, float const*);
SPRK_INST_1 __global__ void sprk_dev::k_deepfm_v2_joint<2, 1, 1, 2, 1, 8, true>(sprk_dev::V2JRun, int const*, float const*, float*, int, int*, float const*);
SPRK_INST_1 __global__ void sprk_dev::k_deepfm_v2_joint<2, 2, 1, 2, 1, 8, false>(sprk_dev::V2JRun, int const*, float const*, float*, int, int*, float const*);
SPRK_INST_1 __global__ void sprk_dev::k_deepfm_v2_joint<2, 2, 1, 2, 1, 8, true>(sprk_dev::V2JRun, int const*, float const*, float*, int, int*, float const*);
SPRK_INST_1 __global__ void sprk_dev::k_deepfm_v2_joint<2, 3, 1, 2, 1, 8, false>(sprk_dev::V2JRun, int const*, float const*, float*, int, int*, float const*);
SPRK_INST_1 __global__ void sprk_dev::k_deepfm_v2_joint<2, 3, 1, 2, 1, 8, true>(sprk_dev::V2JRun, int const*, float const*, float*, int, int*, float const*);
SPRK_INST_1 __global__ void sprk_dev::k_deepfm_v2_joint<3, 1, 1, 2, 1, 8, false>(sprk_dev::V2JRun, int const*, float const*, float*, int, int*, float const*);
SPRK_INST_1 __global__ void sprk_dev::k_deepfm_v2_joint<3, 1, 1, 2, 1, 8, true>(sprk_dev::V2JRun, int const*, float const*, float*, int, int*, float const*);
SPRK_INST_1 __global__ void sprk_dev::k_deepfm_v2_joint<3, 2, 1, 2, 1, 8, false>(sprk_dev::V2JRun, int const*, float const*, float*, int, int*, float const*);
SPRK_INST_1 __global__ void sprk_dev::k_deepfm_v2_joint<3, 2, 1, 2, 1, 8, true>(sprk_dev::V2JRun, int const*, float const*, float*, int, int*, float const*);
SPRK_INST_1 __global__ void sprk_dev::k_deepfm_v2_joint<3, 3, 1, 2, 1, 8, false>(sprk_dev::V2JRun, int const*, float const*, float*, int, int*, float const*);
SPRK_INST_1 __global__ void sprk_dev::k_deepfm_v2_joint<3, 3, 1, 2, 1, 8, true>(sprk_dev::V2JRun, int const*, float const*, float*, int, int*, float const*);
SPRK_INST_1 __global__ void sprk_dev::k_deepfm_v2_joint_many<1, 1, 1, 2, 1, 8, false>(sprk_dev::V2JRun, sprk_dev::V2JMany, int, int*, float const*);
SPRK_INST_1 __global__ void sprk_dev::k_deepfm_v2_joint_many<1, 1, 1, 2, 1, 8, true>(sprk_dev::V2JRun, sprk_dev::V2JMany, int, int*, float const*);
SPRK_INST_1 __global__ void sprk_dev::k_deepfm_v2_joint_many<1, 2, 1, 2, 1, 8, false>(sprk_dev::V2JRun, sprk_dev::V2JMany, int, int*, float const*);
SPRK_INST_1 __global__ void sprk_dev::k_deepfm_v2_joint_many<1, 2, 1, 2, 1, 8, true>(sprk_dev::V2JRun, sprk_dev::V2JMany, int, int*, float const*);
SPRK_INST_1 __global__ void sprk_dev::k_deepfm_v2_joint_many<1, 3, 1, 2, 1, 8, false>(sprk_dev::V2JRun, sprk_dev::V2JMany, int, int*, float const*);
SPRK_INST_1 __global__ void sprk_dev::k_deepfm_v2_joint_many<1, 3, 1, 2, 1, 8, true>(sprk_dev::V2JRun, sprk_dev::V2JMany, int, int*, float const*);
SPRK_INST_1 __global__ void sprk_dev::k_deepfm_v2_joint_many<2, 1, 1, 2, 1, 8, false>(sprk_dev::V2JRun, sprk_dev::V2JMany, int, int*, float const*);
SPRK_INST_1 __global__ void sprk_dev::k_deepfm_v2_joint_many<2, 1, 1, 2, 1, 8, true>(sprk_dev::V2JRun, sprk_dev::V2JMany, int, int*, float const*);
SPRK_INST_1 __global__ void sprk_dev::k_deepfm_v2_joint_many<2, 2, 1, 2, 1, 8, false>(sprk_dev::V2JRun, sprk_dev::V2JMany, int, int*, float const*);
SPRK_INST_1 __global__ void sprk_dev::k_deepfm_v2_joint_many<2, 2, 1, 2, 1, 8, true>(sprk_dev::V2JRun, sprk_dev::V2JMany, int, int*, float const*);
SPRK_INST_1 __global__ void sprk_dev::k_deepfm_v2_joint_many<2, 3, 1, 2, 1, 8, false>(sprk_dev::V2JRun, sprk_dev::V2JMany, int, int*, float const*);
SPRK_INST_1 __global__ void sprk_dev::k_deepfm_v2_joint_many<2, 3, 1, 2, 1, 8, true>(sprk_dev::V2JRun, sprk_dev::V2JMany, int, int*, float const*);
SPRK_INST_1 __global__ void sprk_dev::k_deepfm_v2_joint_many<3, 1, 1, 2, 1, 8, false>(sprk_dev::V2JRun, sprk_dev::V2JMany, int, int*, float const*);
SPRK_INST_1 __global__ void sprk_dev::k_deepfm_v2_joint_many<3, 1, 1, 2, 1, 8, true>(sprk_dev::V2JRun, sprk_dev::V2JMany, int, int*, float const*);
SPRK_INST_1 __global__ void sprk_dev::k_deepfm_v2_joint_many<3, 2, 1, 2, 1, 8, false>(sprk_dev::V2JRun, sprk_dev::V2JMany, int, int*, float const*);
SPRK_INST_1 __global__ void sprk_dev::k_deepfm_v2_joint_many<3, 2, 1, 2, 1, 8, true>(sprk_dev::V2JRun, sprk_dev::V2JMany, int, int*, float const*);
SPRK_INST_1 __global__ void sprk_dev::k_deepfm_v2_joint_many<3, 3, 1, 2, 1, 8, false>(sprk_dev::V2JRun, sprk_dev::V2JMany, int, int*, float const*);
SPRK_INST_1 __global__ void sprk_dev::k_deepfm_v2_joint_many<3, 3, 1, 2, 1, 8, true>(sprk_dev::V2JRun, sprk_dev::V2JMany, int, int*, float const*);
SPRK_INST_2 __global__ void sprk_dev::k_deepfm_v2_joint1<1, 1, false>(sprk_dev::V2JRun, int const*, float const*, float*, int, int*, float const*);
SPRK_INST_2 __global__ void sprk_dev::k_deepfm_v2_joint1<1, 1, true>(sprk_dev::V2JRun, int const*, float const*, float*, int, int*, float const*);
SPRK_INST_2 __global__ void sprk_dev::k_deepfm_v2_joint1<1, 2, false>(sprk_dev::V2JRun, int const*, float const*, float*, int, int*, float const*);
SPRK_INST_2 __global__ void sprk_dev::k_deepfm_v2_joint1<1, 2, true>(sprk_dev::V2JRun, int const*, float const*, float*, int, int*, float const*);
SPRK_INST_2 __global__ void sprk_dev::k_deepfm_v2_joint1<1, 3, false>(sprk_dev::V2JRun, int const*, float const*, float*, int, int*, float const*);
SPRK_INST_2 __global__ void sprk_dev::k_deepfm_v2_joint1<1, 3, true>(sprk_dev::V2JRun, int const*, float const*, float*, int, int*, float const*);
SPRK_INST_2 __global__ void sprk_dev::k_deepfm_v2_joint1<2, 1, false>(sprk_dev::V2JRun, int const*, float const*, float*, int, int*, float const*);
SPRK_INST_2 __global__ void sprk_dev::k_deepfm_v2_joint1<2, 1, true>(sprk_dev::V2JRun, int const*, float const*, float*, int, int*, float const*);
SPRK_INST_2 __global__ void sprk_dev::k_deepfm_v2_joint1<2, 2, false>(sprk_dev::V2JRun, int const*, float const*, float*, int, int*, float const*);
SPRK_INST_2 __global__ void sprk_dev::k_deepfm_v2_joint1<2, 2, true>(sprk_dev::V2JRun, int const*, float const*, float*, int, int*, float const*);
SPRK_INST_2 __global__ void sprk_dev::k_deepfm_v2_joint1<2, 3, false>(sprk_dev::V2JRun, int const*, float const*, float*, int, int*, float const*);
SPRK_INST_2 __global__ void sprk_dev::k_deepfm_v2_joint1<2, 3, true>(sprk_dev::V2JRun, int const*, float const*, float*, int, int*, float const*);
SPRK_INST_2 __global__ void sprk_dev::k_deepfm_v2_joint1<3, 1, false>(sprk_dev::V2JRun, int const*, float const*, float*, int, int*, float const*);
SPRK_INST_2 __global__ void sprk_dev::k_deepfm_v2_joint1<3, 1, true>(sprk_dev::V2JRun, int const*, float const*, float*, int, int*, float const*);
SPRK_INST_2 __global__ void sprk_dev::k_deepfm_v2_joint1<3, 2, false>(sprk_dev::V2JRun, int const*, float const*, float*, int, int*, float const*);
SPRK_INST_2 __global__ void sprk_dev::k_deepfm_v2_joint1<3, 2, true>(sprk_dev::V2JRun, int const*, float const*, float*, int, int*, float const*);
SPRK_INST_2 __global__ void sprk_dev::k_deepfm_v2_joint1<3, 3, false>(sprk_dev::V2JRun, int const*, float const*, float*, int, int*, float const*);
SPRK_INST_2 __global__ void sprk_dev::k_deepfm_v2_joint1<3, 3, true>(sprk_dev::V2JRun, int const*, float const*, float*, int, int*, float const*);
SPRK_INST_2 __global__ void sprk_dev::k_rows_chain<0, 1, 1, 2, 0, false, 8, false>(sprk_dev::RowsRun, int const*, float const*, float*, int, int*, float const*);
SPRK_INST_2 __global__ void sprk_dev::k_rows_chain<1, 2, 1, 3, 3, true, 8, false>(sprk_dev::RowsRun, int const*, float const*, float*, int, int*, float const*);
SPRK_INST_2 __global__ void sprk_dev::k_rows_chain<2, 2, 1, 2, 2, true, 8, false>(sprk_dev::RowsRun, int const*, float const*, float*, int, int*, float const*);
SPRK_INST_2 __global__ void sprk_dev::k_rows_chain<2, 2, 1, 2, 2, true, 8, true>(sprk_dev::RowsRun, int const*, float const*, float*, int, int*, float const*);
SPRK_INST_2 __global__ void sprk_dev::k_rows_chain<2, 2, 1, 3, 3, true, 8, false>(sprk_dev::RowsRun, int const*, float const*, float*, int, int*, float const*);
SPRK_INST_2 __global__ void sprk_dev::k_rows_chain<4, 2, 1, 1, 1, true, 8, false>(sprk_dev::RowsRun, int const*, float const*, float*, int, int*, float const*);
SPRK_INST_2 __global__ void sprk_dev::k_rows_chain<4, 2, 1, 1, 1, true, 8, true>(sprk_dev::RowsRun, int const*, float const*, float*, int, int*, float const*);
SPRK_INST_2 __global__ void sprk_dev::k_rows_chain<4, 2, 1, 2, 1, true, 8, false>(sprk_dev::RowsRun, int const*, float const*, float*, int, int*, float const*);
SPRK_INST_2 __global__ void sprk_dev::k_rows_chain<4, 2, 1, 2, 1, true, 8, true>(sprk_dev::RowsRun, int const*, float const*, float*, int, int*, float const*);
SPRK_INST_2 __global__ void sprk_dev::k_rows_chain<4, 2, 1, 2, 2, true, 8, false>(sprk_dev::RowsRun, int const*, float const*, float*, int, int*, float const*);
SPRK_INST_2 __global__ void sprk_dev::k_rows_chain<4, 2, 1, 2, 2, true, 8, true>(sprk_dev::RowsRun, int const*, float const*, float*, int, int*, float const*);
SPRK_INST_2 __global__ void sprk_dev::k_rows_chain<4, 2, 1, 3, 1, true, 8, false>(sprk_dev::RowsRun, int const*, float const*, float*, int, int*, float const*);
SPRK_INST_2 __global__ void sprk_dev::k_rows_chain<4, 2, 1, 3, 3, true, 8, false>(sprk_dev::RowsRun, int const*, float const*, float*, int, int*, float const*);
SPRK_INST_2 __global__ void sprk_dev::k_rows_chain1<0, 1, 1, 2, 0, false, 8, false>(sprk_dev::RowsRun, int const*, float const*, float*, int, int*, float const*);
SPRK_INST_2 __global__ void sprk_dev::k_rows_chain1<1, 2, 1, 3, 3, true, 8, false>(sprk_dev::RowsRun, int const*, float const*, float*, int, int*, float const*);
SPRK_INST_2 __global__ void sprk_dev::k_rows_chain1<2, 2, 1, 2, 2, true, 8, false>(sprk_dev::RowsRun, int const*, float const*, float*, int, int*, float const*);
SPRK_INST_2 __global__ void sprk_dev::k_rows_chain1<2, 2, 1, 2, 2, true, 8, true>(sprk_dev::RowsRun, int const*, float const*, float*, int, int*, float const*);
SPRK_INST_2 __global__ void sprk_dev::k_rows_chain1<2, 2, 1, 3, 3, true, 8, false>(sprk_dev::RowsRun, int const*, float const*, float*, int, int*, float const*);
SPRK_INST_2 __global__ void sprk_dev::k_rows_chain1<4, 2, 1, 1, 1, true, 8, false>(sprk_dev::RowsRun, int const*, float const*, float*, int, int*, float const*);
SPRK_INST_2 __global__ void sprk_dev::k_rows_chain1<4, 2, 1, 1, 1, true, 8, true>(sprk_dev::RowsRun, int const*, float const*, float*, int, int*, float const*);
SPRK_INST_2 __global__ void sprk_dev::k_rows_chain1<4, 2, 1, 2, 1, true, 8, false>(sprk_dev::RowsRun, int const*, float const*, float*, int, int*, float const*);
SPRK_INST_2 __global__ void sprk_dev::k_rows_chain1<4, 2, 1, 2, 1, true, 8, true>(sprk_dev::RowsRun, int const*, float const*, float*, int, int*, float const*);
SPRK_INST_2 __global__ void sprk_dev::k_rows_chain1<4, 2, 1, 2, 2, true, 8, false>(sprk_dev::RowsRun, int const*, float const*, float*, int, int*, float const*);
SPRK_INST_2 __global__ void sprk_dev::k_rows_chain1<4, 2, 1, 2, 2, true, 8, true>(sprk_dev::RowsRun, int const*, float const*, float*, int, int*, float const*);
SPRK_INST_2 __global__ void sprk_dev::k_rows_chain1<4, 2, 1, 3, 1, true, 8, false>(sprk_dev::RowsRun, int const*, float const*, float*, int, int*, float const*);
SPRK_INST_2 __global__ void sprk_dev::k_rows_chain1<4, 2, 1, 3, 3, true, 8, false>(sprk_dev::RowsRun, int const*, float const*, float*, int, int*, float const*);
SPRK_INST_2 __global__ void sprk_dev::k_rows_chain_many<0, 1, 1, 2, 0, false, 8, false>(sprk_dev::RowsRun, sprk_dev::RowsMany, int, int*, float const*);
SPRK_INST_2 __global__ void sprk_dev::k_rows_chain_many<1, 2, 1, 3, 3, true, 8, false>(sprk_dev::RowsRun, sprk_dev::RowsMany, int, int*, float const*);
SPRK_INST_2 __global__ void sprk_dev::k_rows_chain_many<2, 2, 1, 2, 2, true, 8, false>(sprk_dev::RowsRun, sprk_dev::RowsMany, int, int*, float const*);
SPRK_INST_2 __global__ void sprk_dev::k_rows_chain_many<2, 2, 1, 2, 2, true, 8, true>(sprk_dev::RowsRun, sprk_dev::RowsMany, int, int*, float const*);
SPRK_INST_2 __global__ void sprk_dev::k_rows_chain_many<2, 2, 1, 3, 3, true, 8, false>(sprk_dev::RowsRun, sprk_dev::RowsMany, int, int*, float const*);
SPRK_INST_2 __global__ void sprk_dev::k_rows_chain_many<4, 2, 1, 1, 1, true, 8, false>(sprk_dev::RowsRun, sprk_dev::RowsMany, int, int*, float const*);
SPRK_INST_2 __global__ void sprk_dev::k_rows_chain_many<4, 2, 1, 1, 1, true, 8, true>(sprk_dev::RowsRun, sprk_dev::RowsMany, int, int*, float const*);
SPRK_INST_2 __global__ void sprk_dev::k_rows_chain_many<4, 2, 1, 2, 1, true, 8, false>(sprk_dev::RowsRun, sprk_dev::RowsMany, int, int*, float const*);
SPRK_INST_2 __global__ void sprk_dev::k_rows_chain_many<4, 2, 1, 2, 1, true, 8, true>(sprk_dev::RowsRun, sprk_dev::RowsMany, int, int*, float const*);
SPRK_INST_2 __global__ void sprk_dev::k_rows_chain_many<4, 2, 1, 2, 2, true, 8, false>(sprk_dev::RowsRun, sprk_dev::RowsMany, int, int*, float const*);
SPRK_INST_2 __global__ void sprk_dev::k_rows_chain_many<4, 2, 1, 2, 2, true, 8, true>(sprk_dev::RowsRun, sprk_dev::RowsMany, int, int*, float const*);
SPRK_INST_2 __global__ void sprk_dev::k_rows_chain_many<4, 2, 1, 3, 1, true, 8, false>(sprk_dev::RowsRun, sprk_dev::RowsMany, int, int*, float const*);
SPRK_INST_2 __global__ void sprk_dev::k_rows_chain_many<4, 2, 1, 3, 3, true, 8, false>(sprk_dev::RowsRun, sprk_dev::RowsMany, int, int*, float const*);
SPRK_INST_2 __global__ void sprk_dev::k_v2_pack_image<2, 4, 1, 2, 1, true>(sprk_dev::V2Args, float*);
SPRK_INST_2 __global__ void sprk_dev::k_v2_pack_image<3, 4, 1, 2, 1, true>(sprk_dev::V2Args, float*);
SPRK_INST_2 __global__ void sprk_dev::k_v2_pack_image<4, 4, 1, 2, 1, true>(sprk_dev::V2Args, float*);
SPRK_INST_2 __global__ void sprk_dev::k_v2_pack_image<5, 4, 1, 2, 1, true>(sprk_dev::V2Args, float*);
SPRK_INST_2 __global__ void sprk_dev::k_v2_pack_image<6, 4, 1, 2, 1, true>(sprk_dev::V2Args, float*);
SPRK_INST_3 __global__ void sprk_dev::k_deepfm_pairs<4, 16, 4, 4, 8, false, false>(sprk_dev::V1Run, int const*, float const*, float*, int, int*);
SPRK_INST_3 __global__ void sprk_dev::k_deepfm_pairs<4, 16, 4, 4, 8, false, true>(sprk_dev::V1Run, int const*, float const*, float*, int, int*);
SPRK_INST_3 __global__ void sprk_dev::k_deepfm_pairs<4, 16, 4, 4, 8, true, false>(sprk_dev::V1Run, int const*, float const*, float*, int, int*);
SPRK_INST_3 __global__ void sprk_dev::k_deepfm_pairs<4, 16, 4, 4, 8, true, true>(sprk_dev::V1Run, int const*, float const*, float*, int, int*);
SPRK_INST_3 __global__ void sprk_dev::k_deepfm_pairs<4, 3, 4, 4, 8, false, false>(sprk_dev::V1Run, int const*, float const*, float*, int, int*);
SPRK_INST_3 __global__ void sprk_dev::k_deepfm_pairs<4, 3, 4, 4, 8, false, true>(sprk_dev::V1Run, int const*, float const*, float*, int, int*);
SPRK_INST_3 __global__ void sprk_dev::k_deepfm_pairs<4, 3, 4, 4, 8, true, false>(sprk_dev::V1Run, int const*, float const*, float*, int, int*);
SPRK_INST_3 __global__ void sprk_dev::k_deepfm_pairs<4, 3, 4, 4, 8, true, true>(sprk_dev::V1Run, int const*, float const*, float*, int, int*);
SPRK_INST_3 __global__ void sprk_dev::k_deepfm_pairs<4, 4, 4, 4, 8, false, false>(sprk_dev::V1Run, int const*, float const*, float*, int, int*);
SPRK_INST_3 __global__ void sprk_dev::k_deepfm_pairs<4, 4, 4, 4, 8, false, true>(sprk_dev::V1Run, int const*, float const*, float*, int, int*);
SPRK_INST_3 __global__ void sprk_dev::k_deepfm_pairs<4, 4, 4, 4, 8, true, false>(sprk_dev::V1Run, int const*, float const*, float*, int, int*);
SPRK_INST_3 __global__ void sprk_dev::k_deepfm_pairs<4, 4, 4, 4, 8, true, true>(sprk_dev::V1Run, int const*, float const*, float*, int, int*);
SPRK_INST_3 __global__ void sprk_dev::k_deepfm_pairs<6, 4, 4, 4, 8, false, false>(sprk_dev::V1Run, int const*, float const*, float*, int, int*);
SPRK_INST_3 __global__ void sprk_dev::k_deepfm_pairs<6, 4, 4, 4, 8, false, true>(sprk_dev::V1Run, int const*, float const*, float*, int, int*);
SPRK_INST_3 __global__ void sprk_dev::k_deepfm_pairs<6, 4, 4, 4, 8, true, false>(sprk_dev::V1Run, int const*, float const*, float*, int, int*);
SPRK_INST_3 __global__ void sprk_dev::k_deepfm_pairs<6, 4, 4, 4, 8, true, true>(sprk_dev::V1Run, int const*, float const*, float*, int, int*);
SPRK_INST_3 __global__ void sprk_dev::k_deepfm_pairs1<4, 3, 4, 4, 8, false>(sprk_dev::V1Run, int const*, float const*, float*, int, int*);
SPRK_INST_3 __global__ void sprk_dev::k_deepfm_pairs1<4, 3, 4, 4, 8, true>(sprk_dev::V1Run, int const*, float const*, float*, int, int*);
SPRK_INST_3 __global__ void sprk_dev::k_deepfm_pairs1<4, 4, 4, 4, 8, false>(sprk_dev::V1Run, int const*, float const*, float*, int, int*);
SPRK_INST_3 __global__ void sprk_dev::k_deepfm_pairs1<4, 4, 4, 4, 8, true>(sprk_dev::V1Run, int const*, float const*, float*, int, int*);
SPRK_INST_3 __global__ void sprk_dev::k_deepfm_pairs1<6, 4, 4, 4, 8, false>(sprk_dev::V1Run, int const*, float const*, float*, int, int*);
SPRK_INST_3 __global__ void sprk_dev::k_deepfm_pairs1<6, 4, 4, 4, 8, true>(sprk_dev::V1Run, int const*, float const*, float*, int, int*);
SPRK_INST_3 __global__ void sprk_dev::k_deepfm_pairs_many<4, 16, 4, 4, 8, false, false>(sprk_dev::V1Run, sprk_dev::V1Many, int, int*);
SPRK_INST_3 __global__ void sprk_dev::k_deepfm_pairs_many<4, 16, 4, 4, 8, false, true>(sprk_dev::V1Run, sprk_dev::V1Many, int, int*);
SPRK_INST_3 __global__ void sprk_dev::k_deepfm_pairs_many<4, 16, 4, 4, 8, true, false>(sprk_dev::V1Run, sprk_dev::V1Many, int, int*);
SPRK_INST_3 __global__ void sprk_dev::k_deepfm_pairs_many<4, 16, 4, 4, 8, true, true>(sprk_dev::V1Run, sprk_dev::V1Many, int, int*);
SPRK_INST_3 __global__ void sprk_dev::k_deepfm_pairs_many<4, 3, 4, 4, 8, false, false>(sprk_dev::V1Run, sprk_dev::V1Many, int, int*);
SPRK_INST_3 __global__ void sprk_dev::k_deepfm_pairs_many<4, 3, 4, 4, 8, false, true>(sprk_dev::V1Run, sprk_dev::V1Many, int, int*);
SPRK_INST_3 __global__ void sprk_dev::k_deepfm_pairs_many<4, 3, 4, 4, 8, true, false>(sprk_dev::V1Run, sprk_dev::V1Many, int, int*);
SPRK_INST_3 __global__ void sprk_dev::k_deepfm_pairs_many<4, 3, 4, 4, 8, true, true>(sprk_dev::V1Run, sprk_dev::V1Many, int, int*);
SPRK_INST_3 __global__ void sprk_dev::k_deepfm_pairs_many<4, 4, 4, 4, 8, false, false>(sprk_dev::V1Run, sprk_dev::V1Many, int, int*);
SPRK_INST_3 __global__ void sprk_dev::k_deepfm_pairs_many<4, 4, 4, 4, 8, false, true>(sprk_dev::V1Run, sprk_dev::V1Many, int, int*);
SPRK_INST_3 __global__ void sprk_dev::k_deepfm_pairs_many<4, 4, 4, 4, 8, true, false>(sprk_dev::V1Run, sprk_dev::V1Many, int, int*);
SPRK_INST_3 __global__ void sprk_dev::k_deepfm_pairs_many<4, 4, 4, 4, 8, true, true>(sprk_dev::V1Run, sprk_dev::V1Many, int, int*);
SPRK_INST_3 __global__ void sprk_dev::k_deepfm_pairs_many<6, 4, 4, 4, 8, false, false>(sprk_dev::V1Run, sprk_dev::V1Many, int, int*);
SPRK_INST_3 __global__ void sprk_dev::k_deepfm_pairs_many<6, 4, 4, 4, 8, false, true>(sprk_dev::V1Run, sprk_dev::V1Many, int, int*);
SPRK_INST_3 __global__ void sprk_dev::k_deepfm_pairs_many<6, 4, 4, 4, 8, true, false>(sprk_dev::V1Run, sprk_dev::V1Many, int, int*);
SPRK_INST_3 __global__ void sprk_dev::k_deepfm_pairs_many<6, 4, 4, 4, 8, true, true>(sprk_dev::V1Run, sprk_dev::V1Many, int, int*);
SPRK_INST_3 __global__ void sprk_dev::k_v1_pack_image<4, 4, 1>(sprk_dev::V1Run, float*);
SPRK_INST_3 __global__ void sprk_dev::k_v1_pack_image<4, 4, 4>(sprk_dev::V1Run, float*);
SPRK_INST_4 __global__ void sprk_dev::k_dien_fused<10, 32, 8, 4>(sprk_dev::DienRun, sprk_dev::DinTailRun, int const*, float const*, float*, int, int*, float const*, float*);
SPRK_INST_4 __global__ void sprk_dev::k_dien_fused<16, 32, 8, 4>(sprk_dev::DienRun, sprk_dev::DinTailRun, int const*, float const*, float*, int, int*, float const*, float*);
SPRK_INST_4 __global__ void sprk_dev::k_dien_mfma_pack<10, 32>(float const*, unsigned int const*, float*, int);
SPRK_INST_4 __global__ void sprk_dev::k_dien_mfma_pack<16, 32>(float const*, unsigned int const*, float*, int);
SPRK_INST_4 __global__ void sprk_dev::k_dien_seq<10, 32>(sprk_dev::DienRun, int const*, float*, int, int*);
SPRK_INST_4 __global__ void sprk_dev::k_dien_seq<16, 32>(sprk_dev::DienRun, int const*, float*, int, int*);
SPRK_INST_4 __global__ void sprk_dev::k_dien_seq_mfma<10, 32>(sprk_dev::DienRun, int const*, float*, int, int*);
SPRK_INST_4 __global__ void sprk_dev::k_dien_seq_mfma<16, 32>(sprk_dev::DienRun, int const*, float*, int, int*);
SPRK_INST_4 __global__ void sprk_dev::k_din_attn_cols<1, false>(sprk_dev::DinColsRun, int const*, float*, float*, int, int*, sprk_dev::DinColsArg<false>::type);
SPRK_INST_4 __global__ void sprk_dev::k_din_attn_cols<1, true>(sprk_dev::DinColsRun, int const*, float*, float*, int, int*, sprk_dev::DinColsArg<true>::type);
SPRK_INST_4 __global__ void sprk_dev::k_din_attn_cols<2, false>(sprk_dev::DinColsRun, int const*, float*, float*, int, int*, sprk_dev::DinColsArg<false>::type);
SPRK_INST_4 __global__ void sprk_dev::k_din_attn_cols<2, true>(sprk_dev::DinColsRun, int const*, float*, float*, int, int*, sprk_dev::DinColsArg<true>::type);
SPRK_INST_4 __global__ void sprk_dev::k_din_tail<4, 2, 1, 16, true, false, true>(sprk_dev::DinTailRun, int const*, float const*, float const*, float*, int, int*, float const*, sprk_dev::DinTailMany);
SPRK_INST_4 __global__ void sprk_dev::k_din_tail<4, 2, 1, 16, true, true, true>(sprk_dev::DinTailRun, int const*, float const*, float const*, float*, int, int*, float const*, sprk_dev::DinTailMany);
SPRK_INST_4 __global__ void sprk_dev::k_din_tail<4, 2, 1, 8, false, false, false>(sprk_dev::DinTailRun, int const*, float const*, float const*, float*, int, int*, float const*, sprk_dev::DinTailMany);
SPRK_INST_4 __global__ void sprk_dev::k_din_tail<4, 2, 1, 8, false, true, false>(sprk_dev::DinTailRun, int const*, float const*, float const*, float*, int, int*, float const*, sprk_dev::DinTailMany);
SPRK_INST_4 __global__ void sprk_dev::k_din_tail<4, 2, 1, 8, true, false, false>(sprk_dev::DinTailRun, int const*, float const*, float const*, float*, int, int*, float const*, sprk_dev::DinTailMany);
SPRK_INST_4 __global__ void sprk_dev::k_din_tail<4, 2, 1, 8, true, true, false>(sprk_dev::DinTailRun, int const*, float const*, float const*, float*, int, int*, float const*, sprk_dev::DinTailMany);
SPRK_INST_4 __global__ void sprk_dev::k_din_tail<4, 2, 2, 8, false, false, false>(sprk_dev::DinTailRun, int const*, float const*, float const*, float*, int, int*, float const*, sprk_dev::DinTailMany);
SPRK_INST_4 __global__ void sprk_dev::k_din_tail<4, 2, 2, 8, false, true, false>(sprk_dev::DinTailRun, int const*, float const*, float const*, float*, int, int*, float const*, sprk_dev::DinTailMany);
SPRK_INST_4 __global__ void sprk_dev::k_din_tail<4, 2, 2, 8, true, false, false>(sprk_dev::DinTailRun, int const*, float const*, float const*, float*, int, int*, float const*, sprk_dev::DinTailMany);
SPRK_INST_4 __global__ void sprk_dev::k_din_tail<4, 2, 2, 8, true, false, true>(sprk_dev::DinTailRun, int const*, float const*, float const*, float*, int, int*, float const*, sprk_dev::DinTailMany);
SPRK_INST_4 __global__ void sprk_dev::k_din_tail<4, 2, 2, 8, true, true, false>(sprk_dev::DinTailRun, int const*, float const*, float const*, float*, int, int*, float const*, sprk_dev::DinTailMany);
SPRK_INST_4 __global__ void sprk_dev::k_din_tail<4, 2, 2, 8, true, true, true>(sprk_dev::DinTailRun, int const*, float const*, float const*, float*, int, int*, float const*, sprk_dev::DinTailMany);
SPRK_INST_4 __global__ void sprk_dev::k_din_tail<8, 4, 1, 16, true, false, true>(sprk_dev::DinTailRun, int const*, float const*, float const*, float*, int, int*, float const*, sprk_dev::DinTailMany);
SPRK_INST_4 __global__ void sprk_dev::k_din_tail<8, 4, 1, 16, true, true, true>(sprk_dev::DinTailRun, int const*, float const*, float const*, float*, int, int*, float const*, sprk_dev::DinTailMany);
SPRK_INST_4 __global__ void sprk_dev::k_din_tail<8, 4, 1, 8, false, false, false>(sprk_dev::DinTailRun, int const*, float const*, float const*, float*, int, int*, float const*, sprk_dev::DinTailMany);
SPRK_INST_4 __global__ void sprk_dev::k_din_tail<8, 4, 1, 8, false, true, false>(sprk_dev::DinTailRun, int const*, float const*, float const*, float*, int, int*, float const*, sprk_dev::DinTailMany);
SPRK_INST_4 __global__ void sprk_dev::k_din_tail<8, 4, 1, 8, true, false, false>(sprk_dev::DinTailRun, int const*, float const*, float const*, float*, int, int*, float const*, sprk_dev::DinTailMany);
SPRK_INST_4 __global__ void sprk_dev::k_din_tail<8, 4, 1, 8, true, true, false>(sprk_dev::DinTailRun, int const*, float const*, float const*, float*, int, int*, float const*, sprk_dev::DinTailMany);
SPRK_INST_4 __global__ void sprk_dev::k_din_tail<8, 4, 2, 8, false, false, false>(sprk_dev::DinTailRun, int const*, float const*, float const*, float*, int, int*, float const*, sprk_dev::DinTailMany);
SPRK_INST_4 __global__ void sprk_dev::k_din_tail<8, 4, 2, 8, false, true, false>(sprk_dev::DinTailRun, int const*, float const*, float const*, float*, int, int*, float const*, sprk_dev::DinTailMany);
SPRK_INST_4 __global__ void sprk_dev::k_din_tail<8, 4, 2, 8, true, false, false>(sprk_dev::DinTailRun, int const*, float const*, float const*, float*, int, int*, float const*, sprk_dev::DinTailMany);
SPRK_INST_4 __global__ void sprk_dev::k_din_tail<8, 4, 2, 8, true, false, true>(sprk_dev::DinTailRun, int const*, float const*, float const*, float*, int, int*, float const*, sprk_dev::DinTailMany);
SPRK_INST_4 __global__ void sprk_dev::k_din_tail<8, 4, 2, 8, true, true, false>(sprk_dev::DinTailRun, int const*, float const*, float const*, float*, int, int*, float const*, sprk_dev::DinTailMany);
SPRK_INST_4 __global__ void sprk_dev::k_din_tail<8, 4, 2, 8, true, true, true>(sprk_dev::DinTailRun, int const*, float const*, float const*, float*, int, int*, float const*, sprk_dev::DinTailMany);
SPRK_INST_4 __global__ void sprk_dev::k_din_tail_pack<4, 2, 1>(float const*, int, int, int, int, int, float const*, float const*, float const*, int, float const*, float const*, float const*, int, float const*, float*, float const*, float const*);
SPRK_INST_4 __global__ void sprk_dev::k_din_tail_pack<4, 2, 2>(float const*, int, int, int, int, int, float const*, float const*, float const*, int, float const*, float const*, float const*, int, float const*, float*, float const*, float const*);
SPRK_INST_4 __global__ void sprk_dev::k_din_tail_pack<8, 4, 1>(float const*, int, int, int, int, int, float const*, float const*, float const*, int, float const*, float const*, float const*, int, float const*, float*, float const*, float const*);
SPRK_INST_4 __global__ void sprk_dev::k_din_tail_pack<8, 4, 2>(float const*, int, int, int, int, int, float const*, float const*, float const*, int, float const*, float const*, float const*, int, float const*, float*, float const*, float const*);
SPRK_INST_5 __global__ void sprk_dev::k_din_fused<1, false, false, false>(sprk_dev::DinFusedRun, int const*, float const*, float*, float*, int, int*, sprk_dev::DinFusedArg<false>::type);
SPRK_INST_5 __global__ void sprk_dev::k_din_fused<1, false, false, true>(sprk_dev::DinFusedRun, int const*, float const*, float*, float*, int, int*, sprk_dev::DinFusedArg<false>::type);
SPRK_INST_5 __global__ void sprk_dev::k_din_fused<1, false, true, false>(sprk_dev::DinFusedRun, int const*, float const*, float*, float*, int, int*, sprk_dev::DinFusedArg<false>::type);
SPRK_INST_5 __global__ void sprk_dev::k_din_fused<1, true, false, false>(sprk_dev::DinFusedRun, int const*, float const*, float*, float*, int, int*, sprk_dev::DinFusedArg<true>::type);
SPRK_INST_5 __global__ void sprk_dev::k_din_fused<1, true, true, false>(sprk_dev::DinFusedRun, int const*, float const*, float*, float*, int, int*, sprk_dev::DinFusedArg<true>::type);
SPRK_INST_5 __global__ void sprk_dev::k_din_fused<2, false, false, false>(sprk_dev::DinFusedRun, int const*, float const*, float*, float*, int, int*, sprk_dev::DinFusedArg<false>::type);
SPRK_INST_5 __global__ void sprk_dev::k_din_fused<2, false, false, true>(sprk_dev::DinFusedRun, int const*, float const*, float*, float*, int, int*, sprk_dev::DinFusedArg<false>::type);
SPRK_INST_5 __global__ void sprk_dev::k_din_fused<2, false, true, false>(sprk_dev::DinFusedRun, int const*, float const*, float*, float*, int, int*, sprk_dev::DinFusedArg<false>::type);
SPRK_INST_5 __global__ void sprk_dev::k_din_fused<2, true, false, false>(sprk_dev::DinFusedRun, int const*, float const*, float*, float*, int, int*, sprk_dev::DinFusedArg<true>::type);
SPRK_INST_5 __global__ void sprk_dev::k_din_fused<2, true, true, false>(sprk_dev::DinFusedRun, int const*, float const*, float*, float*, int, int*, sprk_dev::DinFusedArg<true>::type);
SPRK_INST_6 __global__ void sprk_dev::k_mlp_rows<8, 8, 1, -1, 8, false, 0>(sprk_dev::MlpRowsRun, int const*, float const*, float*, int, int*, float const*);
SPRK_INST_6 __global__ void sprk_dev::k_mlp_rows<8, 8, 1, -1, 8, false, 1>(sprk_dev::MlpRowsRun, int const*, float const*, float*, int, int*, float const*);
SPRK_INST_6 __global__ void sprk_dev::k_mlp_rows<8, 8, 1, -1, 8, false, 2>(sprk_dev::MlpRowsRun, int const*, float const*, float*, int, int*, float const*);
SPRK_INST_6 __global__ void sprk_dev::k_mlp_rows<8, 8, 1, -1, 8, true, 0>(sprk_dev::MlpRowsRun, int const*, float const*, float*, int, int*, float const*);
SPRK_INST_6 __global__ void sprk_dev::k_mlp_rows<8, 8, 1, -1, 8, true, 1>(sprk_dev::MlpRowsRun, int const*, float const*, float*, int, int*, float const*);
SPRK_INST_6 __global__ void sprk_dev::k_mlp_rows<8, 8, 1, -1, 8, true, 2>(sprk_dev::MlpRowsRun, int const*, float const*, float*, int, int*, float const*);
SPRK_INST_6 __global__ void sprk_dev::k_mlp_rows<8, 8, 2, -1, 8, false, 0>(sprk_dev::MlpRowsRun, int const*, float const*, float*, int, int*, float const*);
SPRK_INST_6 __global__ void sprk_dev::k_mlp_rows<8, 8, 2, -1, 8, false, 1>(sprk_dev::MlpRowsRun, int const*, float const*, float*, int, int*, float const*);
SPRK_INST_6 __global__ void sprk_dev::k_mlp_rows<8, 8, 2, -1, 8, false, 2>(sprk_dev::MlpRowsRun, int const*, float const*, float*, int, int*, float const*);
SPRK_INST_6 __global__ void sprk_dev::k_mlp_rows<8, 8, 2, -1, 8, true, 0>(sprk_dev::MlpRowsRun, int const*, float const*, float*, int, int*, float const*);
SPRK_INST_6 __global__ void sprk_dev::k_mlp_rows<8, 8, 2, -1, 8, true, 1>(sprk_dev::MlpRowsRun, int const*, float const*, float*, int, int*, float const*);
SPRK_INST_6 __global__ void sprk_dev::k_mlp_rows<8, 8, 2, -1, 8, true, 2>(sprk_dev::MlpRowsRun, int const*, float const*, float*, int, int*, float const*);
SPRK_INST_6 __global__ void sprk_dev::k_mlp_rows<8, 8, 2, 8, 8, true, 0>(sprk_dev::MlpRowsRun, int const*, float const*, float*, int, int*, float const*);
SPRK_INST_6 __global__ void sprk_dev::k_mlp_rows<8, 8, 2, 8, 8, true, 1>(sprk_dev::MlpRowsRun, int const*, float const*, float*, int, int*, float const*);
SPRK_INST_6 __global__ void sprk_dev::k_mlp_rows<8, 8, 2, 8, 8, true, 2>(sprk_dev::MlpRowsRun, int const*, float const*, float*, int, int*, float const*);
SPRK_INST_6 __global__ void sprk_dev::k_mlp_rows_many<8, 8, 1, -1, 8, true, 0>(sprk_dev::MlpRowsRun, sprk_dev::MlpRowsMany, int, int*, float const*);
SPRK_INST_6 __global__ void sprk_dev::k_mlp_rows_many<8, 8, 1, -1, 8, true, 1>(sprk_dev::MlpRowsRun, sprk_dev::MlpRowsMany, int, int*, float const*);
SPRK_INST_6 __global__ void sprk_dev::k_mlp_rows_many<8, 8, 1, -1, 8, true, 2>(sprk_dev::MlpRowsRun, sprk_dev::MlpRowsMany, int, int*, float const*);
SPRK_INST_6 __global__ void sprk_dev::k_mlp_rows_many<8, 8, 2, -1, 8, true, 0>(sprk_dev::MlpRowsRun, sprk_dev::MlpRowsMany, int, int*, float const*);
SPRK_INST_6 __global__ void sprk_dev::k_mlp_rows_many<8, 8, 2, -1, 8, true, 1>(sprk_dev::MlpRowsRun, sprk_dev::MlpRowsMany, int, int*, float const*);
SPRK_INST_6 __global__ void sprk_dev::k_mlp_rows_many<8, 8, 2, -1, 8, true, 2>(sprk_dev::MlpRowsRun, sprk_dev::MlpRowsMany, int, int*, float const*);
SPRK_INST_6 __global__ void sprk_dev::k_mlp_rows_many<8, 8, 2, 8, 8, true, 0>(sprk_dev::MlpRowsRun, sprk_dev::MlpRowsMany, int, int*, float const*);
SPRK_INST_6 __global__ void sprk_dev::k_mlp_rows_many<8, 8, 2, 8, 8, true, 1>(sprk_dev::MlpRowsRun, sprk_dev::MlpRowsMany, int, int*, float const*);
SPRK_INST_6 __global__ void sprk_dev::k_mlp_rows_many<8, 8, 2, 8, 8, true, 2>(sprk_dev::MlpRowsRun, sprk_dev::MlpRowsMany, int, int*, float const*);
SPRK_INST_6 __global__ void sprk_dev::k_mlp_rows_pack<8, 8, false>(float const*, int, int, int, float const*, float const*, int, float const*, float const*, int, float const*, float*);
SPRK_INST_6 __global__ void sprk_dev::k_mlp_rows_pack<8, 8, true>(float const*, int, int, int, float const*, float const*, int, float const*, float const*, int, float const*, float*);
#endif
```

Baseline: 16.90 billion.

## Stage small-vocabulary embedding tables in LDS for DeepFM pairs kernel

Fields whose vocabulary is at most 31 are reordered to the end, and their embedding rows plus first-order weights are packed into an extra LDS region next to the weight image. The kernel then reads those rows from shared memory instead of gathering them from global memory. New template variants carry the small-field count, and the setup falls back to the old variants when none match. The aim is to cut global gather traffic, at the cost of more LDS per workgroup (which may lower occupancy) and more kernel instantiations.

```diff
diff --git a/sparrowrecsys_amd/csrc/api_forward.h b/sparrowrecsys_amd/csrc/api_forward.h
--- a/sparrowrecsys_amd/csrc/api_forward.h
+++ b/sparrowrecsys_amd/csrc/api_forward.h
@@ -483,8 +483,12 @@
     }
     site(cols, "din_attn");
     site(h->stage == Stage::DienSeqMfma, "dien_seq");
-    const int n = snprintf(buf, buf_bytes, "kernel=%s;stage=%s;stage_waves_per_workgroup=%d;fused=%d;uploaded_bytes=%zu;derived_bytes=%zu;first_dense_fold=%d;split_f16=%s;build_defines=%s", kern,
-                           kStageName[(int)h->stage], cols ? DC_WAVES : 0, h->route != Route::Tile ? 1 : 0, uploaded, h->derived_bytes, h->n_acc_folded, split, SPRK_BUILD_DEFINES_STR);
+    char ldsf[48] = "";
+    if (h->route == Route::Pairs)
+        for (int j = 0; j < h->v1_run.ns; ++j)
+            snprintf(ldsf + strlen(ldsf), sizeof(ldsf) - strlen(ldsf), j ? ",%d" : "%d", h->v1_run.col[h->v1_run.nf - h->v1_run.ns + j]);
+    const int n = snprintf(buf, buf_bytes, "kernel=%s;stage=%s;stage_waves_per_workgroup=%d;fused=%d;uploaded_bytes=%zu;derived_bytes=%zu;first_dense_fold=%d;split_f16=%s;lds_fields=%s;build_defines=%s", kern,
+                           kStageName[(int)h->stage], cols ? DC_WAVES : 0, h->route != Route::Tile ? 1 : 0, uploaded, h->derived_bytes, h->n_acc_folded, split, ldsf, SPRK_BUILD_DEFINES_STR);
     if (n < 0 || (size_t)n >= buf_bytes) return fail(SPRK_EINVAL, "describe: buffer of %zu bytes is too small", buf_bytes);
     return SPRK_OK;
 }
diff --git a/sparrowrecsys_amd/csrc/host_common.h b/sparrowrecsys_amd/csrc/host_common.h
--- a/sparrowrecsys_amd/csrc/host_common.h
+++ b/sparrowrecsys_amd/csrc/host_common.h
@@ -79,6 +79,7 @@
     bool dyn_f16 = true;
     bool v1_chain = true;
     bool v1_one = true;
+    bool v1_small_lds = true;
     bool mlp_chain = true;
     bool vmm_tables = true;
     bool din_tail = true;
@@ -105,6 +106,7 @@
         t.half_range_guard = !off("SPRK_HALF_RANGE_GUARD"); t.dyn_f16 = !off("SPRK_DYN_F16");
         t.v1_chain = !off("SPRK_V1_CHAIN");
         t.v1_one = !off("SPRK_V1_ONE");
+        t.v1_small_lds = !off("SPRK_V1_SMALL_LDS");
         t.mlp_chain = !off("SPRK_MLP_CHAIN");
         t.vmm_tables = !off("SPRK_VMM_TABLES");
         t.din_tail = !off("SPRK_DIN_TAIL"); t.din_legacy = on("SPRK_DIN_LEGACY"); t.din_half = !off("SPRK_DIN_HALF");
diff --git a/sparrowrecsys_amd/csrc/host_setup_pairs.h b/sparrowrecsys_amd/csrc/host_setup_pairs.h
--- a/sparrowrecsys_amd/csrc/host_setup_pairs.h
+++ b/sparrowrecsys_amd/csrc/host_setup_pairs.h
@@ -2,51 +2,51 @@
 constexpr int V1_ONE_MAX_TASKS = 16384;
 typedef void (*V1LaunchFn)(const V1Run&, const int*, const float*, float*, int, int*, int, hipStream_t);
 typedef void (*V1LaunchManyFn)(const V1Run&, const V1Many&, int, int*, int, hipStream_t);
-template <int NF, int NV, bool SEP>
+template <int NF, int NV, int NS, bool SEP>
 void v1_launch(const V1Run& a, const int* ids, const float* dense, float* out, int B, int* err, int grid, hipStream_t st) {
-    const size_t lds = V1Lds<4, 4, (NV + 3) / 4>::bytes;
+    const size_t lds = V1Lds<4, 4, (NV + 3) / 4>::bytes + sizeof(float) * (NS ? a.small_floats : 0);
     if (a.inv_w1_scale != 0.f)
-        hipLaunchKernelGGL((k_deepfm_pairs<NF, NV, 4, 4, V1_WAVES, true, SEP>), dim3(grid), dim3(V1_WAVES * 64), lds, st, a, ids, dense, out, B, err);
+        hipLaunchKernelGGL((k_deepfm_pairs<NF, NV, NS, 4, 4, V1_WAVES, true, SEP>), dim3(grid), dim3(V1_WAVES * 64), lds, st, a, ids, dense, out, B, err);
     else
-        hipLaunchKernelGGL((k_deepfm_pairs<NF, NV, 4, 4, V1_WAVES, false, SEP>), dim3(grid), dim3(V1_WAVES * 64), lds, st, a, ids, dense, out, B, err);
-}
-template <int NF, int NV, bool SEP>
+        hipLaunchKernelGGL((k_deepfm_pairs<NF, NV, NS, 4, 4, V1_WAVES, false, SEP>), dim3(grid), dim3(V1_WAVES * 64), lds, st, a, ids, dense, out, B, err);
+}
+template <int NF, int NV, int NS, bool SEP>
 void v1_launch_one(const V1Run& a, const int* ids, const float* dense, float* out, int B, int* err, int grid, hipStream_t st) {
     if constexpr (NV <= 4) {
-        const size_t lds = V1Lds<4, 4, 1>::bytes;
-        hipLaunchKernelGGL((k_deepfm_pairs1<NF, NV, 4, 4, V1_WAVES, SEP>), dim3(grid), dim3(V1_WAVES * 64), lds, st, a, ids, dense, out, B, err);
-    }
-}
-template <int NF, int NV, bool SEP>
+        const size_t lds = V1Lds<4, 4, 1>::bytes + sizeof(float) * (NS ? a.small_floats : 0);
+        hipLaunchKernelGGL((k_deepfm_pairs1<NF, NV, NS, 4, 4, V1_WAVES, SEP>), dim3(grid), dim3(V1_WAVES * 64), lds, st, a, ids, dense, out, B, err);
+    }
+}
+template <int NF, int NV, int NS, bool SEP>
 void v1_launch_many(const V1Run& a, const V1Many& m, int B, int* err, int grid, hipStream_t st) {
-    const size_t lds = V1Lds<4, 4, (NV + 3) / 4>::bytes;
+    const size_t lds = V1Lds<4, 4, (NV + 3) / 4>::bytes + sizeof(float) * (NS ? a.small_floats : 0);
     if (a.inv_w1_scale != 0.f)
-        hipLaunchKernelGGL((k_deepfm_pairs_many<NF, NV, 4, 4, V1_WAVES, true, SEP>), dim3(grid), dim3(V1_WAVES * 64), lds, st, a, m, B, err);
+        hipLaunchKernelGGL((k_deepfm_pairs_many<NF, NV, NS, 4, 4, V1_WAVES, true, SEP>), dim3(grid), dim3(V1_WAVES * 64), lds, st, a, m, B, err);
     else
-        hipLaunchKernelGGL((k_deepfm_pairs_many<NF, NV, 4, 4, V1_WAVES, false, SEP>), dim3(grid), dim3(V1_WAVES * 64), lds, st, a, m, B, err);
-}
-template <int NF, int NV, bool SEP>
+        hipLaunchKernelGGL((k_deepfm_pairs_many<NF, NV, NS, 4, 4, V1_WAVES, false, SEP>), dim3(grid), dim3(V1_WAVES * 64), lds, st, a, m, B, err);
+}
+template <int NF, int NV, int NS, bool SEP>
 int v1_prepare(const V1Run& r, float* img) {
     constexpr int PC = (NV + 3) / 4;
     hipLaunchKernelGGL((k_v1_pack_image<4, 4, PC>), dim3(1), dim3(256), 0, 0, r, img);
     HIP_TRY(hipGetLastError());
-    const size_t lds = V1Lds<4, 4, PC>::bytes;
-    HIP_TRY(hipFuncSetAttribute(reinterpret_cast<const void*>(&k_deepfm_pairs<NF, NV, 4, 4, V1_WAVES, true, SEP>), hipFuncAttributeMaxDynamicSharedMemorySize, (int)lds));
-    HIP_TRY(hipFuncSetAttribute(reinterpret_cast<const void*>(&k_deepfm_pairs<NF, NV, 4, 4, V1_WAVES, false, SEP>), hipFuncAttributeMaxDynamicSharedMemorySize, (int)lds));
-    HIP_TRY(hipFuncSetAttribute(reinterpret_cast<const void*>(&k_deepfm_pairs_many<NF, NV, 4, 4, V1_WAVES, true, SEP>), hipFuncAttributeMaxDynamicSharedMemorySize, (int)lds));
-    HIP_TRY(hipFuncSetAttribute(reinterpret_cast<const void*>(&k_deepfm_pairs_many<NF, NV, 4, 4, V1_WAVES, false, SEP>), hipFuncAttributeMaxDynamicSharedMemorySize, (int)lds));
+    const size_t lds = V1Lds<4, 4, PC>::bytes + sizeof(float) * V1Lds<4, 4, PC>::small_max(NS);
+    HIP_TRY(hipFuncSetAttribute(reinterpret_cast<const void*>(&k_deepfm_pairs<NF, NV, NS, 4, 4, V1_WAVES, true, SEP>), hipFuncAttributeMaxDynamicSharedMemorySize, (int)lds));
+    HIP_TRY(hipFuncSetAttribute(reinterpret_cast<const void*>(&k_deepfm_pairs<NF, NV, NS, 4, 4, V1_WAVES, false, SEP>), hipFuncAttributeMaxDynamicSharedMemorySize, (int)lds));
+    HIP_TRY(hipFuncSetAttribute(reinterpret_cast<const void*>(&k_deepfm_pairs_many<NF, NV, NS, 4, 4, V1_WAVES, true, SEP>), hipFuncAttributeMaxDynamicSharedMemorySize, (int)lds));
+    HIP_TRY(hipFuncSetAttribute(reinterpret_cast<const void*>(&k_deepfm_pairs_many<NF, NV, NS, 4, 4, V1_WAVES, false, SEP>), hipFuncAttributeMaxDynamicSharedMemorySize, (int)lds));
     if constexpr (NV <= 4)
-        HIP_TRY(hipFuncSetAttribute(reinterpret_cast<const void*>(&k_deepfm_pairs1<NF, NV, 4, 4, V1_WAVES, SEP>), hipFuncAttributeMaxDynamicSharedMemorySize, (int)lds));
+        HIP_TRY(hipFuncSetAttribute(reinterpret_cast<const void*>(&k_deepfm_pairs1<NF, NV, NS, 4, 4, V1_WAVES, SEP>), hipFuncAttributeMaxDynamicSharedMemorySize, (int)lds));
     return SPRK_OK;
 }
-struct V1Variant { int nf, nv; bool sep; V1LaunchFn launch; V1LaunchFn launch_one; V1LaunchManyFn launch_many; int (*prepare)(const V1Run&, float*); size_t lds_bytes; };
-#define V1_VARIANT(NF, NV, SEP) {NF, NV, SEP, &v1_launch<NF, NV, SEP>, &v1_launch_one<NF, NV, SEP>, &v1_launch_many<NF, NV, SEP>, &v1_prepare<NF, NV, SEP>, V1Lds<4, 4, (NV + 3) / 4>::bytes}
-#define V1_BOTH(NF, NV) V1_VARIANT(NF, NV, true), V1_VARIANT(NF, NV, false)
+struct V1Variant { int nf, nv, ns; bool sep; V1LaunchFn launch; V1LaunchFn launch_one; V1LaunchManyFn launch_many; int (*prepare)(const V1Run&, float*); size_t lds_bytes; };
+#define V1_VARIANT(NF, NV, NS, SEP) {NF, NV, NS, SEP, &v1_launch<NF, NV, NS, SEP>, &v1_launch_one<NF, NV, NS, SEP>, &v1_launch_many<NF, NV, NS, SEP>, &v1_prepare<NF, NV, NS, SEP>, V1Lds<4, 4, (NV + 3) / 4>::bytes}
+#define V1_BOTH(NF, NV, NS) V1_VARIANT(NF, NV, 0, true), V1_VARIANT(NF, NV, 0, false), V1_VARIANT(NF, NV, NS, true), V1_VARIANT(NF, NV, NS, false)
 const V1Variant kV1Variants[] = {
-    V1_BOTH(6, 4),
-    V1_BOTH(4, 3),
-    V1_BOTH(4, 4),
-    V1_BOTH(4, 16),
+    V1_BOTH(6, 4, 3),
+    V1_BOTH(4, 3, 2),
+    V1_BOTH(4, 4, 2),
+    V1_BOTH(4, 16, 2),
 };
 
 int setup_deepfm_pairs(sprk_engine* h) {
@@ -145,11 +145,16 @@
             order[no++] = twin;
         }
     }
-    for (int f = 0; f < nf; ++f) {
-        bool deep = false;
-        for (int i = 0; i < r.n_deep; ++i) deep |= order[i] == f;
-        if (!deep) order[no++] = f;
-    }
+    int n_small = 0;
+    for (int pass = 0; pass < 2; ++pass)
+        for (int f = 0; f < nf; ++f) {
+            bool deep = false;
+            for (int i = 0; i < r.n_deep; ++i) deep |= order[i] == f;
+            const bool small = !deep && r.vocab[f] <= V1_SMALL_VOCAB;
+            if (deep || small != (pass == 1)) continue;
+            order[no++] = f;
+            n_small += small;
+        }
     {
         V1Run t = r;
         int inv[V1_MAX_FIELDS];
@@ -173,9 +178,12 @@
     for (int d = 0; d < n_dsep; ++d) r.table[nf + d] = dsep_tab[d];
     const float* const* deep_tables = sep ? &r.table[nf] : &r.table[0];
     int variant = -1;
-    for (size_t v = 0; v < sizeof(kV1Variants) / sizeof(kV1Variants[0]); ++v)
-        if (kV1Variants[v].nf == nf && kV1Variants[v].nv == Dp / 4 && kV1Variants[v].sep == sep) variant = (int)v;
+    for (int want : {h->tune.v1_small_lds ? n_small : 0, 0}) {
+        for (size_t v = 0; v < sizeof(kV1Variants) / sizeof(kV1Variants[0]) && variant < 0; ++v)
+            if (kV1Variants[v].nf == nf && kV1Variants[v].nv == Dp / 4 && kV1Variants[v].sep == sep && kV1Variants[v].ns == want) variant = (int)v;
+    }
     if (variant < 0) return SPRK_OK;
+    r.ns = kV1Variants[variant].ns;
     const int H0 = o0.N, H1 = o1.N;
     const float* W0 = (const float*)h->slot_ptr[o0.w_slot];
     const int PC = (Dp / 4 + 3) / 4;
@@ -204,9 +212,20 @@
         if (frag && frag0) { r.w1frag = frag; r.inv_w1_scale = 1.0f / w_scale; r.w0frag = frag0; r.inv_w0_scale = 1.0f / w0_scale; }
     }
     {
+        const int SS = 16 * PC + 4, img_floats = (int)(kV1Variants[variant].lds_bytes / sizeof(float));
+        int sf = 0;
+        for (int j = 0; j < r.ns; ++j) { r.s_off[j] = sf; sf += (r.vocab[nf - r.ns + j] + 1) * SS; }
+        r.small_floats = (sf + 255) & ~255;
         float* img = nullptr;
-        SPRK_TRY(dev_alloc(h, &img, kV1Variants[variant].lds_bytes));
+        SPRK_TRY(dev_alloc(h, &img, kV1Variants[variant].lds_bytes + (size_t)r.small_floats * sizeof(float)));
         SPRK_TRY(kV1Variants[variant].prepare(r, img));
+        if (r.small_floats) HIP_TRY(hipMemset(img + img_floats, 0, (size_t)r.small_floats * sizeof(float)));
+        for (int j = 0; j < r.ns; ++j) {
+            const int f = nf - r.ns + j, rows = r.vocab[f] + 1;
+            hipLaunchKernelGGL(k_v1_build_small, dim3((rows * SS + 255) / 256), dim3(256), 0, 0, r.table[f], Dp, r.w1[f], rows, SS,
+                               img + img_floats + r.s_off[j]);
+        }
+        HIP_TRY(hipGetLastError());
         HIP_TRY(hipDeviceSynchronize());
         r.image = img;
     }
diff --git a/sparrowrecsys_amd/csrc/k_chain_v1.h b/sparrowrecsys_amd/csrc/k_chain_v1.h
--- a/sparrowrecsys_amd/csrc/k_chain_v1.h
+++ b/sparrowrecsys_amd/csrc/k_chain_v1.h
@@ -2,6 +2,8 @@
 #define V1_MAX_FIELDS 8
 #define V1_MAX_DEEP 2
 #define V1_MAX_ROWS (V1_MAX_FIELDS + V1_MAX_DEEP)
+#define V1_MAX_SMALL 3
+#define V1_SMALL_VOCAB 31
 
 struct V1Run {
     int F, ND, n_num;
@@ -32,7 +34,18 @@
     float e_scale, e_inv;
     const float* tab;
     unsigned rowbase[V1_MAX_ROWS];
+    int ns;
+    int s_off[V1_MAX_SMALL];
+    int small_floats;
 };
+
+static __global__ __launch_bounds__(256) void k_v1_build_small(const float* __restrict__ table, int Dp, const float* __restrict__ w1, int rows,
+                                                        int SS, float* __restrict__ out) {
+    for (int i = blockIdx.x * 256 + threadIdx.x; i < rows * SS; i += gridDim.x * 256) {
+        const int v = i / SS, c = i - v * SS;
+        out[i] = c < Dp ? table[(size_t)v * Dp + c] : (c == SS - 4 ? w1[v] : 0.f);
+    }
+}
 
 static __global__ __launch_bounds__(256) void k_v1_build_rows(const float* __restrict__ table, int Dp, const float* __restrict__ w1,
                                                        long long rows, float* __restrict__ out, const float* __restrict__ deep, int deep_off) {
@@ -85,6 +98,9 @@
     static constexpr int total = off_hd + H1;
     static constexpr int total_pad = (total + 255) & ~255;
     static constexpr size_t bytes = sizeof(float) * total_pad;
+    static constexpr int SS = 16 * PC + 4;
+    static constexpr int small_max(int ns) { return (ns * (V1_SMALL_VOCAB + 1) * SS + 255) & ~255; }
+    static_assert(2 * (bytes + sizeof(float) * small_max(V1_MAX_SMALL)) <= 160 * 1024, "two workgroups per CU");
     static_assert(H1C * (H0C / 2) * 512 <= H1 * S1 && H0C * PC * 512 <= H0 * SE && H0C % 2 == 0, "fragments fit their regions");
 };
 
@@ -115,21 +131,24 @@
     for (int i = tid; i < LD::H1; i += 256) { img[LD::off_b1 + i] = A.b1[i]; img[LD::off_hd + i] = A.hdeep[i]; }
 }
 
-template <int NR, int PC>
+template <int NR, int PC, int NS>
 struct V1Set {
     f32x4 x[NR][PC];
     float xa, xb;
     float w1a, w1b;
+    int so[NS ? NS : 1];
 };
 
-template <int NF, int NV, int H0C, int H1C, int WAVES, bool DYN, bool MB, bool SEP, bool ONE = false>
+template <int NF, int NV, int NS, int H0C, int H1C, int WAVES, bool DYN, bool MB, bool SEP, bool ONE = false>
 __device__ __forceinline__ void v1_body(const V1Run& A, const int* __restrict__ ids0, const float* __restrict__ dense0,
                                         float* __restrict__ out0, int B, int* __restrict__ err, const V1Many* __restrict__ Mp) {
     constexpr int PC = (NV + 3) / 4;
-    constexpr int NR = NF + (SEP ? V1_MAX_DEEP : 0);
-    constexpr int DB = SEP ? NF : 0;
+    constexpr int NG = NF - NS;
+    constexpr int NR = NG + (SEP ? V1_MAX_DEEP : 0);
+    constexpr int DB = SEP ? NG : 0;
     using LD = V1Lds<H0C, H1C, PC>;
-    using Set = V1Set<NR, PC>;
+    using Set = V1Set<NR, PC, NS>;
+    static_assert(NS >= 0 && NS <= V1_MAX_SMALL && NG >= 2 && (NS == 0 || NG <= 4), "small fields: the deep fields are gathered, w1b's fields are all small");
     static_assert(!(ONE && MB) && !(ONE && PC > 1), "one-task shape: one batch, narrow rows");
     static_assert(NF >= 2 && NF <= V1_MAX_FIELDS && NV >= 1 && (NV <= 4 || NV % 4 == 0) && NV <= 16, "shape");
     const int tid = threadIdx.x;
@@ -177,41 +196,46 @@
             bad |= (unsigned)(idv[f] + 1) > (unsigned)A.vocab[f];
             sid[f] = min((unsigned)idv[f], (unsigned)A.vocab[f]);
         }
+#pragma unroll
+        for (int j = 0; j < NS; ++j) {
+            S.so[j] = LD::total_pad + A.s_off[j] + (int)sid[NG + j] * LD::SS;
+            asm volatile("" : "+v"(S.so[j]));
+        }
         if ((ONE && NV == 4) || (PC == 1 && A.tab)) {
             const char* tb = reinterpret_cast<const char*>(A.tab);
-            unsigned ro[NF];
-#pragma unroll
-            for (int f = 0; f < NF; ++f) ro[f] = (sid[f] + A.rowbase[f]) * 128u;
-#pragma unroll
-            for (int f = 0; f < NF; ++f) S.x[f][0] = q < NV ? *reinterpret_cast<const f32x4*>(tb + (ro[f] + 16u * q)) : zero;
+            unsigned ro[NG];
+#pragma unroll
+            for (int f = 0; f < NG; ++f) ro[f] = (sid[f] + A.rowbase[f]) * 128u;
+#pragma unroll
+            for (int f = 0; f < NG; ++f) S.x[f][0] = q < NV ? *reinterpret_cast<const f32x4*>(tb + (ro[f] + 16u * q)) : zero;
             if constexpr (SEP) {
 #pragma unroll
                 for (int d = 0; d < V1_MAX_DEEP; ++d) {
-                    S.x[NF + d][0] = zero;
+                    S.x[NG + d][0] = zero;
                     if (d < A.n_deep) {
                         const unsigned rd = A.pack ? ro[d] + (unsigned)A.pack : (sid[d] + A.rowbase[NF + d]) * 128u;
-                        if (q < NV) S.x[NF + d][0] = *reinterpret_cast<const f32x4*>(tb + (rd + 16u * q));
+                        if (q < NV) S.x[NG + d][0] = *reinterpret_cast<const f32x4*>(tb + (rd + 16u * q));
                     }
                 }
             }
-            unsigned oa = ro[0], ob = ro[NF > 4 ? 4 : 0];
-            if (NF > 1) oa = q == 1 ? ro[NF > 1 ? 1 : 0] : oa;
-            if (NF > 2) oa = q == 2 ? ro[NF > 2 ? 2 : 0] : oa;
-            if (NF > 3) oa = q == 3 ? ro[NF > 3 ? 3 : 0] : oa;
-            if (NF > 5) ob = q == 1 ? ro[NF > 5 ? 5 : 0] : ob;
-            if (NF > 6) ob = q == 2 ? ro[NF > 6 ? 6 : 0] : ob;
-            if (NF > 7) ob = q == 3 ? ro[NF > 7 ? 7 : 0] : ob;
+            unsigned oa = ro[0], ob = ro[NG > 4 ? 4 : 0];
+            if (NG > 1) oa = q == 1 ? ro[NG > 1 ? 1 : 0] : oa;
+            if (NG > 2) oa = q == 2 ? ro[NG > 2 ? 2 : 0] : oa;
+            if (NG > 3) oa = q == 3 ? ro[NG > 3 ? 3 : 0] : oa;
+            if (NG > 5) ob = q == 1 ? ro[NG > 5 ? 5 : 0] : ob;
+            if (NG > 6) ob = q == 2 ? ro[NG > 6 ? 6 : 0] : ob;
+            if (NG > 7) ob = q == 3 ? ro[NG > 7 ? 7 : 0] : ob;
             const float* pa = reinterpret_cast<const float*>(tb + (oa + 64u));
             if (A.w1c) {
                 const unsigned ci = (q == 1 ? sid[1] + A.w1cbase[1] : sid[0] + A.w1cbase[0]);
                 pa = q < A.n_deep ? A.w1c + ci : pa;
             }
-            S.w1a = (q < NF) ? *pa : 0.f;
-            S.w1b = (NF > 4 && q + 4 < NF) ? *reinterpret_cast<const float*>(tb + (ob + 64u)) : 0.f;
+            S.w1a = (q < NG) ? *pa : 0.f;
+            S.w1b = (NG > 4 && q + 4 < NG) ? *reinterpret_cast<const float*>(tb + (ob + 64u)) : 0.f;
             return;
         }
 #pragma unroll
-        for (int f = 0; f < NF; ++f)
+        for (int f = 0; f < NG; ++f)
 #pragma unroll
             for (int pc = 0; pc < PC; ++pc)
                 S.x[f][pc] = 4 * pc + q < NV ? ld4(A.table[f] + (size_t)sid[f] * A.row_floats + 16 * pc + 4 * q) : zero;
@@ -220,21 +244,21 @@
             for (int d = 0; d < V1_MAX_DEEP; ++d)
 #pragma unroll
                 for (int pc = 0; pc < PC; ++pc)
-                    S.x[NF + d][pc] = (d < A.n_deep && 4 * pc + q < NV) ? ld4(A.table[NF + d] + (size_t)sid[d] * A.row_floats + 16 * pc + 4 * q) : zero;
+                    S.x[NG + d][pc] = (d < A.n_deep && 4 * pc + q < NV) ? ld4(A.table[NF + d] + (size_t)sid[d] * A.row_floats + 16 * pc + 4 * q) : zero;
         }
         {
             const float* pa = A.w1[0] + sid[0];
-            if (NF > 1) pa = q == 1 ? A.w1[NF > 1 ? 1 : 0] + sid[NF > 1 ? 1 : 0] : pa;
-            if (NF > 2) pa = q == 2 ? A.w1[NF > 2 ? 2 : 0] + sid[NF > 2 ? 2 : 0] : pa;
-            if (NF > 3) pa = q == 3 ? A.w1[NF > 3 ? 3 : 0] + sid[NF > 3 ? 3 : 0] : pa;
-            S.w1a = (q < NF) ? *pa : 0.f;
+            if (NG > 1) pa = q == 1 ? A.w1[NG > 1 ? 1 : 0] + sid[NG > 1 ? 1 : 0] : pa;
+            if (NG > 2) pa = q == 2 ? A.w1[NG > 2 ? 2 : 0] + sid[NG > 2 ? 2 : 0] : pa;
+            if (NG > 3) pa = q == 3 ? A.w1[NG > 3 ? 3 : 0] + sid[NG > 3 ? 3 : 0] : pa;
+            S.w1a = (q < NG) ? *pa : 0.f;
             S.w1b = 0.f;
-            if (NF > 4) {
-                const float* pb = A.w1[NF > 4 ? 4 : 0] + sid[NF > 4 ? 4 : 0];
-                if (NF > 5) pb = q == 1 ? A.w1[NF > 5 ? 5 : 0] + sid[NF > 5 ? 5 : 0] : pb;
-                if (NF > 6) pb = q == 2 ? A.w1[NF > 6 ? 6 : 0] + sid[NF > 6 ? 6 : 0] : pb;
-                if (NF > 7) pb = q == 3 ? A.w1[NF > 7 ? 7 : 0] + sid[NF > 7 ? 7 : 0] : pb;
-                S.w1b = (q + 4 < NF) ? *pb : 0.f;
+            if (NG > 4) {
+                const float* pb = A.w1[NG > 4 ? 4 : 0] + sid[NG > 4 ? 4 : 0];
+                if (NG > 5) pb = q == 1 ? A.w1[NG > 5 ? 5 : 0] + sid[NG > 5 ? 5 : 0] : pb;
+                if (NG > 6) pb = q == 2 ? A.w1[NG > 6 ? 6 : 0] + sid[NG > 6 ? 6 : 0] : pb;
+                if (NG > 7) pb = q == 3 ? A.w1[NG > 7 ? 7 : 0] + sid[NG > 7 ? 7 : 0] : pb;
+                S.w1b = (q + 4 < NG) ? *pb : 0.f;
             }
         }
     };
@@ -242,6 +266,24 @@
     auto compute = [&](const Set& S) -> float {
 #pragma clang fp contract(off)
         constexpr bool NUM_FIRST = ONE && NV == 4;
+        f32x4 xs[NS ? NS : 1][PC];
+        float la = 0.f, lb = 0.f;
+        if constexpr (NS > 0) {
+#pragma unroll
+            for (int j = 0; j < NS; ++j)
+#pragma unroll
+                for (int pc = 0; pc < PC; ++pc) xs[j][pc] = ld4(smem + S.so[j] + 16 * pc + 4 * q);
+            int oa = S.so[0], ob = S.so[NF > 4 ? 4 - NG : 0];
+#pragma unroll
+            for (int j = 1; j < NS; ++j) {
+                if (NG + j < 4) oa = q == NG + j ? S.so[j] : oa;
+                if (NG + j > 4) ob = q == NG + j - 4 ? S.so[j] : ob;
+            }
+            la = smem[oa + 16 * PC];
+            if constexpr (NF > 4) lb = smem[ob + 16 * PC];
+            __builtin_amdgcn_sched_barrier(0);
+        }
+        auto X = [&](int f, int pc) -> f32x4 { return f < NG ? S.x[f < NG ? f : 0][pc] : xs[f < NG ? 0 : f - NG][pc]; };
         f32x4 h0[H0C];
         auto deep0_numerics = [&]() {
 #pragma unroll
@@ -263,12 +305,17 @@
                 const f32x2 hw2 = {hw, hw};
 #pragma unroll
                 for (int pc = 0; pc < PC; ++pc) {
-                    const f32x4 xa = S.x[a][pc], xb = S.x[b][pc];
+                    const f32x4 xa = X(a, pc), xb = X(b, pc);
                     pa = __builtin_elementwise_fma(f32x2{xa.x, xa.y} * f32x2{xb.x, xb.y}, hw2, pa);
                     pb = __builtin_elementwise_fma(f32x2{xa.z, xa.w} * f32x2{xb.z, xb.w}, hw2, pb);
                 }
             }
-        float z = (S.w1a + S.w1b) + ((pa[0] + pa[1]) + (pb[0] + pb[1]));
+        float w1a = S.w1a, w1b = S.w1b;
+        if constexpr (NS > 0) {
+            w1a = q < NG ? S.w1a : (q < (NF < 4 ? NF : 4) ? la : 0.f);
+            w1b = (NF > 4 && q + 4 < NF) ? lb : 0.f;
+        }
+        float z = (w1a + w1b) + ((pa[0] + pa[1]) + (pb[0] + pb[1]));
         if constexpr (!NUM_FIRST) deep0_numerics();
         f32x4 ec[2 * PC];
 #pragma unroll
@@ -392,7 +439,8 @@
     if (tA < ntasks) ld_ids(tA, idA);
     if (!ONE && tB < ntasks) ld_ids(tB, idB);
 #pragma unroll 1
-    for (int c = wave; c < LD::total_pad / 256; c += WAVES) lds_dma16(A.image + c * 256 + lane * 4, smem + c * 256);
+    for (int c = wave; c < LD::total_pad / 256 + (NS ? A.small_floats / 256 : 0); c += WAVES)
+        lds_dma16(A.image + c * 256 + lane * 4, smem + c * 256);
     Set SA, SB;
     if constexpr (ONE) {
         __builtin_amdgcn_s_waitcnt(0x0F70);
@@ -433,17 +481,17 @@
     if (__ballot(bad) != 0 && lane == 0) atomicOr(err, 1);
 }
 
-template <int NF, int NV, int H0C, int H1C, int WAVES, bool DYN, bool SEP>
+template <int NF, int NV, int NS, int H0C, int H1C, int WAVES, bool DYN, bool SEP>
 __global__ __launch_bounds__(WAVES * 64, 2) void k_deepfm_pairs(const V1Run A, const int* __restrict__ ids, const float* __restrict__ dense,
                                                                 float* __restrict__ out, int B, int* __restrict__ err) {
-    v1_body<NF, NV, H0C, H1C, WAVES, DYN, false, SEP>(A, ids, dense, out, B, err, nullptr);
-}
-template <int NF, int NV, int H0C, int H1C, int WAVES, bool DYN, bool SEP>
+    v1_body<NF, NV, NS, H0C, H1C, WAVES, DYN, false, SEP>(A, ids, dense, out, B, err, nullptr);
+}
+template <int NF, int NV, int NS, int H0C, int H1C, int WAVES, bool DYN, bool SEP>
 __global__ __launch_bounds__(WAVES * 64, 2) void k_deepfm_pairs_many(const V1Run A, const V1Many M, int B, int* __restrict__ err) {
-    v1_body<NF, NV, H0C, H1C, WAVES, DYN, true, SEP>(A, nullptr, nullptr, nullptr, B, err, &M);
-}
-template <int NF, int NV, int H0C, int H1C, int WAVES, bool SEP>
+    v1_body<NF, NV, NS, H0C, H1C, WAVES, DYN, true, SEP>(A, nullptr, nullptr, nullptr, B, err, &M);
+}
+template <int NF, int NV, int NS, int H0C, int H1C, int WAVES, bool SEP>
 __global__ __launch_bounds__(WAVES * 64, 4) void k_deepfm_pairs1(const V1Run A, const int* __restrict__ ids, const float* __restrict__ dense,
                                                                  float* __restrict__ out, int B, int* __restrict__ err) {
-    v1_body<NF, NV, H0C, H1C, WAVES, true, false, SEP, true>(A, ids, dense, out, B, err, nullptr);
-}
+    v1_body<NF, NV, NS, H0C, H1C, WAVES, true, false, SEP, true>(A, ids, dense, out, B, err, nullptr);
+}
diff --git a/sparrowrecsys_amd/csrc/tu_instances.h b/sparrowrecsys_amd/csrc/tu_instances.h
--- a/sparrowrecsys_amd/csrc/tu_instances.h
+++ b/sparrowrecsys_amd/csrc/tu_instances.h
@@ -130,44 +130,82 @@
 SPRK_INST_2 __global__ void sprk_dev::k_v2_pack_image<4, 4, 1, 2, 1, true>(sprk_dev::V2Args, float*);
 SPRK_INST_2 __global__ void sprk_dev::k_v2_pack_image<5, 4, 1, 2, 1, true>(sprk_dev::V2Args, float*);
 SPRK_INST_2 __global__ void sprk_dev::k_v2_pack_image<6, 4, 1, 2, 1, true>(sprk_dev::V2Args, float*);
-SPRK_INST_3 __global__ void sprk_dev::k_deepfm_pairs<4, 16, 4, 4, 8, false, false>(sprk_dev::V1Run, int const*, float const*, float*, int, int*);
-SPRK_INST_3 __global__ void sprk_dev::k_deepfm_pairs<4, 16, 4, 4, 8, false, true>(sprk_dev::V1Run, int const*, float const*, float*, int, int*);
-SPRK_INST_3 __global__ void sprk_dev::k_deepfm_pairs<4, 16, 4, 4, 8, true, false>(sprk_dev::V1Run, int const*, float const*, float*, int, int*);
-SPRK_INST_3 __global__ void sprk_dev::k_deepfm_pairs<4, 16, 4, 4, 8, true, true>(sprk_dev::V1Run, int const*, float const*, float*, int, int*);
-SPRK_INST_3 __global__ void sprk_dev::k_deepfm_pairs<4, 3, 4, 4, 8, false, false>(sprk_dev::V1Run, int const*, float const*, float*, int, int*);
-SPRK_INST_3 __global__ void sprk_dev::k_deepfm_pairs<4, 3, 4, 4, 8, false, true>(sprk_dev::V1Run, int const*, float const*, float*, int, int*);
-SPRK_INST_3 __global__ void sprk_dev::k_deepfm_pairs<4, 3, 4, 4, 8, true, false>(sprk_dev::V1Run, int const*, float const*, float*, int, int*);
-SPRK_INST_3 __global__ void sprk_dev::k_deepfm_pairs<4, 3, 4, 4, 8, true, true>(sprk_dev::V1Run, int const*, float const*, float*, int, int*);
-SPRK_INST_3 __global__ void sprk_dev::k_deepfm_pairs<4, 4, 4, 4, 8, false, false>(sprk_dev::V1Run, int const*, float const*, float*, int, int*);
-SPRK_INST_3 __global__ void sprk_dev::k_deepfm_pairs<4, 4, 4, 4, 8, false, true>(sprk_dev::V1Run, int const*, float const*, float*, int, int*);
-SPRK_INST_3 __global__ void sprk_dev::k_deepfm_pairs<4, 4, 4, 4, 8, true, false>(sprk_dev::V1Run, int const*, float const*, float*, int, int*);
-SPRK_INST_3 __global__ void sprk_dev::k_deepfm_pairs<4, 4, 4, 4, 8, true, true>(sprk_dev::V1Run, int const*, float const*, float*, int, int*);
-SPRK_INST_3 __global__ void sprk_dev::k_deepfm_pairs<6, 4, 4, 4, 8, false, false>(sprk_dev::V1Run, int const*, float const*, float*, int, int*);
-SPRK_INST_3 __global__ void sprk_dev::k_deepfm_pairs<6, 4, 4, 4, 8, false, true>(sprk_dev::V1Run, int const*, float const*, float*, int, int*);
-SPRK_INST_3 __global__ void sprk_dev::k_deepfm_pairs<6, 4, 4, 4, 8, true, false>(sprk_dev::V1Run, int const*, float const*, float*, int, int*);
-SPRK_INST_3 __global__ void sprk_dev::k_deepfm_pairs<6, 4, 4, 4, 8, true, true>(sprk_dev::V1Run, int const*, float const*, float*, int, int*);
-SPRK_INST_3 __global__ void sprk_dev::k_deepfm_pairs1<4, 3, 4, 4, 8, false>(sprk_dev::V1Run, int const*, float const*, float*, int, int*);
-SPRK_INST_3 __global__ void sprk_dev::k_deepfm_pairs1<4, 3, 4, 4, 8, true>(sprk_dev::V1Run, int const*, float const*, float*, int, int*);
-SPRK_INST_3 __global__ void sprk_dev::k_deepfm_pairs1<4, 4, 4, 4, 8, false>(sprk_dev::V1Run, int const*, float const*, float*, int, int*);
-SPRK_INST_3 __global__ void sprk_dev::k_deepfm_pairs1<4, 4, 4, 4, 8, true>(sprk_dev::V1Run, int const*, float const*, float*, int, int*);
-SPRK_INST_3 __global__ void sprk_dev::k_deepfm_pairs1<6, 4, 4, 4, 8, false>(sprk_dev::V1Run, int const*, float const*, float*, int, int*);
-SPRK_INST_3 __global__ void sprk_dev::k_deepfm_pairs1<6, 4, 4, 4, 8, true>(sprk_dev::V1Run, int const*, float const*, float*, int, int*);
-SPRK_INST_3 __global__ void sprk_dev::k_deepfm_pairs_many<4, 16, 4, 4, 8, false, false>(sprk_dev::V1Run, sprk_dev::V1Many, int, int*);
-SPRK_INST_3 __global__ void sprk_dev::k_deepfm_pairs_many<4, 16, 4, 4, 8, false, true>(sprk_dev::V1Run, sprk_dev::V1Many, int, int*);
-SPRK_INST_3 __global__ void sprk_dev::k_deepfm_pairs_many<4, 16, 4, 4, 8, true, false>(sprk_dev::V1Run, sprk_dev::V1Many, int, int*);
-SPRK_INST_3 __global__ void sprk_dev::k_deepfm_pairs_many<4, 16, 4, 4, 8, true, true>(sprk_dev::V1Run, sprk_dev::V1Many, int, int*);
-SPRK_INST_3 __global__ void sprk_dev::k_deepfm_pairs_many<4, 3, 4, 4, 8, false, false>(sprk_dev::V1Run, sprk_dev::V1Many, int, int*);
-SPRK_INST_3 __global__ void sprk_dev::k_deepfm_pairs_many<4, 3, 4, 4, 8, false, true>(sprk_dev::V1Run, sprk_dev::V1Many, int, int*);
-SPRK_INST_3 __global__ void sprk_dev::k_deepfm_pairs_many<4, 3, 4, 4, 8, true, false>(sprk_dev::V1Run, sprk_dev::V1Many, int, int*);
-SPRK_INST_3 __global__ void sprk_dev::k_deepfm_pairs_many<4, 3, 4, 4, 8, true, true>(sprk_dev::V1Run, sprk_dev::V1Many, int, int*);
-SPRK_INST_3 __global__ void sprk_dev::k_deepfm_pairs_many<4, 4, 4, 4, 8, false, false>(sprk_dev::V1Run, sprk_dev::V1Many, int, int*);
-SPRK_INST_3 __global__ void sprk_dev::k_deepfm_pairs_many<4, 4, 4, 4, 8, false, true>(sprk_dev::V1Run, sprk_dev::V1Many, int, int*);
-SPRK_INST_3 __global__ void sprk_dev::k_deepfm_pairs_many<4, 4, 4, 4, 8, true, false>(sprk_dev::V1Run, sprk_dev::V1Many, int, int*);
-SPRK_INST_3 __global__ void sprk_dev::k_deepfm_pairs_many<4, 4, 4, 4, 8, true, true>(sprk_dev::V1Run, sprk_dev::V1Many, int, int*);
-SPRK_INST_3 __global__ void sprk_dev::k_deepfm_pairs_many<6, 4, 4, 4, 8, false, false>(sprk_dev::V1Run, sprk_dev::V1Many, int, int*);
-SPRK_INST_3 __global__ void sprk_dev::k_deepfm_pairs_many<6, 4, 4, 4, 8, false, true>(sprk_dev::V1Run, sprk_dev::V1Many, int, int*);
-SPRK_INST_3 __global__ void sprk_dev::k_deepfm_pairs_many<6, 4, 4, 4, 8, true, false>(sprk_dev::V1Run, sprk_dev::V1Many, int, int*);
-SPRK_INST_3 __global__ void sprk_dev::k_deepfm_pairs_many<6, 4, 4, 4, 8, true, true>(sprk_dev::V1Run, sprk_dev::V1Many, int, int*);
+SPRK_INST_3 __global__ void sprk_dev::k_deepfm_pairs<4, 16, 0, 4, 4, 8, false, false>(sprk_dev::V1Run, int const*, float const*, float*, int, int*);
+SPRK_INST_3 __global__ void sprk_dev::k_deepfm_pairs<4, 16, 0, 4, 4, 8, false, true>(sprk_dev::V1Run, int const*, float const*, float*, int, int*);
+SPRK_INST_3 __global__ void sprk_dev::k_deepfm_pairs<4, 16, 0, 4, 4, 8, true, false>(sprk_dev::V1Run, int const*, float const*, float*, int, int*);
+SPRK_INST_3 __global__ void sprk_dev::k_deepfm_pairs<4, 16, 0, 4, 4, 8, true, true>(sprk_dev::V1Run, int const*, float const*, float*, int, int*);
+SPRK_INST_3 __global__ void sprk_dev::k_deepfm_pairs<4, 16, 2, 4, 4, 8, false, false>(sprk_dev::V1Run, int const*, float const*, float*, int, int*);
+SPRK_INST_3 __global__ void sprk_dev::k_deepfm_pairs<4, 16, 2, 4, 4, 8, false, true>(sprk_dev::V1Run, int const*, float const*, float*, int, int*);
+SPRK_INST_3 __global__ void sprk_dev::k_deepfm_pairs<4, 16, 2, 4, 4, 8, true, false>(sprk_dev::V1Run, int const*, float const*, float*, int, int*);
+SPRK_INST_3 __global__ void sprk_dev::k_deepfm_pairs<4, 16, 2, 4, 4, 8, true, true>(sprk_dev::V1Run, int const*, float const*, float*, int, int*);
+SPRK_INST_3 __global__ void sprk_dev::k_deepfm_pairs<4, 3, 0, 4, 4, 8, false, false>(sprk_dev::V1Run, int const*, float const*, float*, int, int*);
+SPRK_INST_3 __global__ void sprk_dev::k_deepfm_pairs<4, 3, 0, 4, 4, 8, false, true>(sprk_dev::V1Run, int const*, float const*, float*, int, int*);
+SPRK_INST_3 __global__ void sprk_dev::k_deepfm_pairs<4, 3, 0, 4, 4, 8, true, false>(sprk_dev::V1Run, int const*, float const*, float*, int, int*);
+SPRK_INST_3 __global__ void sprk_dev::k_deepfm_pairs<4, 3, 0, 4, 4, 8, true, true>(sprk_dev::V1Run, int const*, float const*, float*, int, int*);
+SPRK_INST_3 __global__ void sprk_dev::k_deepfm_pairs<4, 3, 2, 4, 4, 8, false, false>(sprk_dev::V1Run, int const*, float const*, float*, int, int*);
+SPRK_INST_3 __global__ void sprk_dev::k_deepfm_pairs<4, 3, 2, 4, 4, 8, false, true>(sprk_dev::V1Run, int const*, float const*, float*, int, int*);
+SPRK_INST_3 __global__ void sprk_dev::k_deepfm_pairs<4, 3, 2, 4, 4, 8, true, false>(sprk_dev::V1Run, int const*, float const*, float*, int, int*);
+SPRK_INST_3 __global__ void sprk_dev::k_deepfm_pairs<4, 3, 2, 4, 4, 8, true, true>(sprk_dev::V1Run, int const*, float const*, float*, int, int*);
+SPRK_INST_3 __global__ void sprk_dev::k_deepfm_pairs<4, 4, 0, 4, 4, 8, false, false>(sprk_dev::V1Run, int const*, float const*, float*, int, int*);
+SPRK_INST_3 __global__ void sprk_dev::k_deepfm_pairs<4, 4, 0, 4, 4, 8, false, true>(sprk_dev::V1Run, int const*, float const*, float*, int, int*);
+SPRK_INST_3 __global__ void sprk_dev::k_deepfm_pairs<4, 4, 0, 4, 4, 8, true, false>(sprk_dev::V1Run, int const*, float const*, float*, int, int*);
+SPRK_INST_3 __global__ void sprk_dev::k_deepfm_pairs<4, 4, 0, 4, 4, 8, true, true>(sprk_dev::V1Run, int const*, float const*, float*, int, int*);
+SPRK_INST_3 __global__ void sprk_dev::k_deepfm_pairs<4, 4, 2, 4, 4, 8, false, false>(sprk_dev::V1Run, int const*, float const*, float*, int, int*);
+SPRK_INST_3 __global__ void sprk_dev::k_deepfm_pairs<4, 4, 2, 4, 4, 8, false, true>(sprk_dev::V1Run, int const*, float const*, float*, int, int*);
+SPRK_INST_3 __global__ void sprk_dev::k_deepfm_pairs<4, 4, 2, 4, 4, 8, true, false>(sprk_dev::V1Run, int const*, float const*, float*, int, int*);
+SPRK_INST_3 __global__ void sprk_dev::k_deepfm_pairs<4, 4, 2, 4, 4, 8, true, true>(sprk_dev::V1Run, int const*, float const*, float*, int, int*);
+SPRK_INST_3 __global__ void sprk_dev::k_deepfm_pairs<6, 4, 0, 4, 4, 8, false, false>(sprk_dev::V1Run, int const*, float const*, float*, int, int*);
+SPRK_INST_3 __global__ void sprk_dev::k_deepfm_pairs<6, 4, 0, 4, 4, 8, false, true>(sprk_dev::V1Run, int const*, float const*, float*, int, int*);
+SPRK_INST_3 __global__ void sprk_dev::k_deepfm_pairs<6, 4, 0, 4, 4, 8, true, false>(sprk_dev::V1Run, int const*, float const*, float*, int, int*);
+SPRK_INST_3 __global__ void sprk_dev::k_deepfm_pairs<6, 4, 0, 4, 4, 8, true, true>(sprk_dev::V1Run, int const*, float const*, float*, int, int*);
+SPRK_INST_3 __global__ void sprk_dev::k_deepfm_pairs<6, 4, 3, 4, 4, 8, false, false>(sprk_dev::V1Run, int const*, float const*, float*, int, int*);
+SPRK_INST_3 __global__ void sprk_dev::k_deepfm_pairs<6, 4, 3, 4, 4, 8, false, true>(sprk_dev::V1Run, int const*, float const*, float*, int, int*);
+SPRK_INST_3 __global__ void sprk_dev::k_deepfm_pairs<6, 4, 3, 4, 4, 8, true, false>(sprk_dev::V1Run, int const*, float const*, float*, int, int*);
+SPRK_INST_3 __global__ void sprk_dev::k_deepfm_pairs<6, 4, 3, 4, 4, 8, true, true>(sprk_dev::V1Run, int const*, float const*, float*, int, int*);
+SPRK_INST_3 __global__ void sprk_dev::k_deepfm_pairs1<4, 3, 0, 4, 4, 8, false>(sprk_dev::V1Run, int const*, float const*, float*, int, int*);
+SPRK_INST_3 __global__ void sprk_dev::k_deepfm_pairs1<4, 3, 0, 4, 4, 8, true>(sprk_dev::V1Run, int const*, float const*, float*, int, int*);
+SPRK_INST_3 __global__ void sprk_dev::k_deepfm_pairs1<4, 3, 2, 4, 4, 8, false>(sprk_dev::V1Run, int const*, float const*, float*, int, int*);
+SPRK_INST_3 __global__ void sprk_dev::k_deepfm_pairs1<4, 3, 2, 4, 4, 8, true>(sprk_dev::V1Run, int const*, float const*, float*, int, int*);
+SPRK_INST_3 __global__ void sprk_dev::k_deepfm_pairs1<4, 4, 0, 4, 4, 8, false>(sprk_dev::V1Run, int const*, float const*, float*, int, int*);
+SPRK_INST_3 __global__ void sprk_dev::k_deepfm_pairs1<4, 4, 0, 4, 4, 8, true>(sprk_dev::V1Run, int const*, float const*, float*, int, int*);
+SPRK_INST_3 __global__ void sprk_dev::k_deepfm_pairs1<4, 4, 2, 4, 4, 8, false>(sprk_dev::V1Run, int const*, float const*, float*, int, int*);
+SPRK_INST_3 __global__ void sprk_dev::k_deepfm_pairs1<4, 4, 2, 4, 4, 8, true>(sprk_dev::V1Run, int const*, float const*, float*, int, int*);
+SPRK_INST_3 __global__ void sprk_dev::k_deepfm_pairs1<6, 4, 0, 4, 4, 8, false>(sprk_dev::V1Run, int const*, float const*, float*, int, int*);
+SPRK_INST_3 __global__ void sprk_dev::k_deepfm_pairs1<6, 4, 0, 4, 4, 8, true>(sprk_dev::V1Run, int const*, float const*, float*, int, int*);
+SPRK_INST_3 __global__ void sprk_dev::k_deepfm_pairs1<6, 4, 3, 4, 4, 8, false>(sprk_dev::V1Run, int const*, float const*, float*, int, int*);
+SPRK_INST_3 __global__ void sprk_dev::k_deepfm_pairs1<6, 4, 3, 4, 4, 8, true>(sprk_dev::V1Run, int const*, float const*, float*, int, int*);
+SPRK_INST_3 __global__ void sprk_dev::k_deepfm_pairs_many<4, 16, 0, 4, 4, 8, false, false>(sprk_dev::V1Run, sprk_dev::V1Many, int, int*);
+SPRK_INST_3 __global__ void sprk_dev::k_deepfm_pairs_many<4, 16, 0, 4, 4, 8, false, true>(sprk_dev::V1Run, sprk_dev::V1Many, int, int*);
+SPRK_INST_3 __global__ void sprk_dev::k_deepfm_pairs_many<4, 16, 0, 4, 4, 8, true, false>(sprk_dev::V1Run, sprk_dev::V1Many, int, int*);
+SPRK_INST_3 __global__ void sprk_dev::k_deepfm_pairs_many<4, 16, 0, 4, 4, 8, true, true>(sprk_dev::V1Run, sprk_dev::V1Many, int, int*);
+SPRK_INST_3 __global__ void sprk_dev::k_deepfm_pairs_many<4, 16, 2, 4, 4, 8, false, false>(sprk_dev::V1Run, sprk_dev::V1Many, int, int*);
+SPRK_INST_3 __global__ void sprk_dev::k_deepfm_pairs_many<4, 16, 2, 4, 4, 8, false, true>(sprk_dev::V1Run, sprk_dev::V1Many, int, int*);
+SPRK_INST_3 __global__ void sprk_dev::k_deepfm_pairs_many<4, 16, 2, 4, 4, 8, true, false>(sprk_dev::V1Run, sprk_dev::V1Many, int, int*);
+SPRK_INST_3 __global__ void sprk_dev::k_deepfm_pairs_many<4, 16, 2, 4, 4, 8, true, true>(sprk_dev::V1Run, sprk_dev::V1Many, int, int*);
+SPRK_INST_3 __global__ void sprk_dev::k_deepfm_pairs_many<4, 3, 0, 4, 4, 8, false, false>(sprk_dev::V1Run, sprk_dev::V1Many, int, int*);
+SPRK_INST_3 __global__ void sprk_dev::k_deepfm_pairs_many<4, 3, 0, 4, 4, 8, false, true>(sprk_dev::V1Run, sprk_dev::V1Many, int, int*);
+SPRK_INST_3 __global__ void sprk_dev::k_deepfm_pairs_many<4, 3, 0, 4, 4, 8, true, false>(sprk_dev::V1Run, sprk_dev::V1Many, int, int*);
+SPRK_INST_3 __global__ void sprk_dev::k_deepfm_pairs_many<4, 3, 0, 4, 4, 8, true, true>(sprk_dev::V1Run, sprk_dev::V1Many, int, int*);
+SPRK_INST_3 __global__ void sprk_dev::k_deepfm_pairs_many<4, 3, 2, 4, 4, 8, false, false>(sprk_dev::V1Run, sprk_dev::V1Many, int, int*);
+SPRK_INST_3 __global__ void sprk_dev::k_deepfm_pairs_many<4, 3, 2, 4, 4, 8, false, true>(sprk_dev::V1Run, sprk_dev::V1Many, int, int*);
+SPRK_INST_3 __global__ void sprk_dev::k_deepfm_pairs_many<4, 3, 2, 4, 4, 8, true, false>(sprk_dev::V1Run, sprk_dev::V1Many, int, int*);
+SPRK_INST_3 __global__ void sprk_dev::k_deepfm_pairs_many<4, 3, 2, 4, 4, 8, true, true>(sprk_dev::V1Run, sprk_dev::V1Many, int, int*);
+SPRK_INST_3 __global__ void sprk_dev::k_deepfm_pairs_many<4, 4, 0, 4, 4, 8, false, false>(sprk_dev::V1Run, sprk_dev::V1Many, int, int*);
+SPRK_INST_3 __global__ void sprk_dev::k_deepfm_pairs_many<4, 4, 0, 4, 4, 8, false, true>(sprk_dev::V1Run, sprk_dev::V1Many, int, int*);
+SPRK_INST_3 __global__ void sprk_dev::k_deepfm_pairs_many<4, 4, 0, 4, 4, 8, true, false>(sprk_dev::V1Run, sprk_dev::V1Many, int, int*);
+SPRK_INST_3 __global__ void sprk_dev::k_deepfm_pairs_many<4, 4, 0, 4, 4, 8, true, true>(sprk_dev::V1Run, sprk_dev::V1Many, int, int*);
+SPRK_INST_3 __global__ void sprk_dev::k_deepfm_pairs_many<4, 4, 2, 4, 4, 8, false, false>(sprk_dev::V1Run, sprk_dev::V1Many, int, int*);
+SPRK_INST_3 __global__ void sprk_dev::k_deepfm_pairs_many<4, 4, 2, 4, 4, 8, false, true>(sprk_dev::V1Run, sprk_dev::V1Many, int, int*);
+SPRK_INST_3 __global__ void sprk_dev::k_deepfm_pairs_many<4, 4, 2, 4, 4, 8, true, false>(sprk_dev::V1Run, sprk_dev::V1Many, int, int*);
+SPRK_INST_3 __global__ void sprk_dev::k_deepfm_pairs_many<4, 4, 2, 4, 4, 8, true, true>(sprk_dev::V1Run, sprk_dev::V1Many, int, int*);
+SPRK_INST_3 __global__ void sprk_dev::k_deepfm_pairs_many<6, 4, 0, 4, 4, 8, false, false>(sprk_dev::V1Run, sprk_dev::V1Many, int, int*);
+SPRK_INST_3 __global__ void sprk_dev::k_deepfm_pairs_many<6, 4, 0, 4, 4, 8, false, true>(sprk_dev::V1Run, sprk_dev::V1Many, int, int*);
+SPRK_INST_3 __global__ void sprk_dev::k_deepfm_pairs_many<6, 4, 0, 4, 4, 8, true, false>(sprk_dev::V1Run, sprk_dev::V1Many, int, int*);
+SPRK_INST_3 __global__ void sprk_dev::k_deepfm_pairs_many<6, 4, 0, 4, 4, 8, true, true>(sprk_dev::V1Run, sprk_dev::V1Many, int, int*);
+SPRK_INST_3 __global__ void sprk_dev::k_deepfm_pairs_many<6, 4, 3, 4, 4, 8, false, false>(sprk_dev::V1Run, sprk_dev::V1Many, int, int*);
+SPRK_INST_3 __global__ void sprk_dev::k_deepfm_pairs_many<6, 4, 3, 4, 4, 8, false, true>(sprk_dev::V1Run, sprk_dev::V1Many, int, int*);
+SPRK_INST_3 __global__ void sprk_dev::k_deepfm_pairs_many<6, 4, 3, 4, 4, 8, true, false>(sprk_dev::V1Run, sprk_dev::V1Many, int, int*);
+SPRK_INST_3 __global__ void sprk_dev::k_deepfm_pairs_many<6, 4, 3, 4, 4, 8, true, true>(sprk_dev::V1Run, sprk_dev::V1Many, int, int*);
 SPRK_INST_3 __global__ void sprk_dev::k_v1_pack_image<4, 4, 1>(sprk_dev::V1Run, float*);
 SPRK_INST_3 __global__ void sprk_dev::k_v1_pack_image<4, 4, 4>(sprk_dev::V1Run, float*);
 SPRK_INST_4 __global__ void sprk_dev::k_dien_fused<10, 32, 8, 4>(sprk_dev::DienRun, sprk_dev::DinTailRun, int const*, float const*, float*, int, int*, float const*, float*);
```

After: 16.21 billion. -4.1%, worse.
